# DJjjjhao/FIRA-ICSE

Measured on AMD Instinct MI355X. Metric: training commits/sec (FIRA default config), higher is better.
Workload: dtype f32; 1 GPU; BASELINE configs[1]: FIRA training step (fwd+bwd+Adam, dropout 0.1/0.2), batch 32 commits/GPU, fp32, 650-node graphs (mean nnz 1066/graph), vocab 24650; global_batch=32, parallelism=dp1

## Files before the change

fira_icse_amd/build.py:

```python
from __future__ import annotations

import os
import subprocess
import sys
from concurrent.futures import ThreadPoolExecutor

HERE = os.path.dirname(os.path.abspath(__file__))
CSRC = os.path.join(HERE, "csrc")
LIB = os.path.join(HERE, "libfira_hip.so")
SOURCES = ["gemm_f32.hip", "gemm_bf16.hip", "gemm_wgrad_panel.hip", "gemm_bf16_panel.hip", "gemm_small.hip", "spmm.hip", "spmm_dense.hip", "gcn_fused.hip", "comb_fused.hip", "head_x3.hip", "rowops.hip", "attention.hip", "copyhead.hip", "beam.hip", "engine.hip", "layout.cpp", "hostlists.cpp"]
HEADERS = ["common.h", "engine.h", "epilogue.h", "mfma_frag.h", "x3.h", os.path.join("..", "..", "include", "fira_hip.h")]
FLAGS = ["--offload-arch=gfx950", "-O3", "-std=c++17", "-fPIC", "-munsafe-fp-atomics", "-Wno-unused-result"]


def _hipcc() -> str:
    for cand in (os.environ.get("HIPCC"), "/opt/rocm/bin/hipcc", "hipcc"):
        if cand and (os.path.isabs(cand) and os.path.exists(cand) or not os.path.isabs(cand)):
            return cand
    raise RuntimeError("hipcc not found")


def build(force: bool = False, verbose: bool = False) -> str:
    objdir = os.path.join(HERE, "build")
    os.makedirs(objdir, exist_ok=True)
    hdr_time = max(os.path.getmtime(os.path.join(CSRC, h)) for h in HEADERS)
    hipcc = _hipcc()
    jobs = []
    for src in SOURCES:
        sp = os.path.join(CSRC, src)
        op = os.path.join(objdir, src + ".o")
        if force or not os.path.exists(op) or os.path.getmtime(op) < max(os.path.getmtime(sp), hdr_time):
            cmd = [hipcc] + FLAGS + (["-x", "hip"] if src.endswith(".cpp") else []) + ["-c", sp, "-o", op]
            jobs.append((src, cmd))

    def run(job):
        src, cmd = job
        if verbose:
            print(" ".join(cmd), flush=True)
        r = subprocess.run(cmd, capture_output=True, text=True)
        if r.returncode != 0:
            raise RuntimeError("hipcc failed on %s:\n%s" % (src, r.stderr[-4000:]))
        return src

    if jobs:
        with ThreadPoolExecutor(max_workers=min(8, len(jobs))) as ex:
            list(ex.map(run, jobs))
    objs = [os.path.join(objdir, s + ".o") for s in SOURCES]
    if jobs or not os.path.exists(LIB):
        cmd = [hipcc, "--offload-arch=gfx950", "-shared", "-fPIC", "-o", LIB] + objs
        r = subprocess.run(cmd, capture_output=True, text=True)
        if r.returncode != 0:
            raise RuntimeError("link failed:\n%s" % r.stderr[-4000:])
    return LIB


if __name__ == "__main__":
    print(build(force="--force" in sys.argv, verbose=True))
```

fira_icse_amd/csrc/comb_fused.hip:

```cpp
#include "engine.h"
#include "mfma_frag.h"
#include "epilogue.h"
#include "x3.h"

namespace fira {

constexpr int CF_TILE = 16;
constexpr int CF_TMAX = 2;
constexpr int CF_ROWS = CF_TILE * CF_TMAX;
constexpr int CF_WAVES = 16;
constexpr int CF_RPW = CF_ROWS / CF_WAVES;
constexpr int CF_GRID = 256;
constexpr size_t CF_LDS = 84 * 1024;

typedef float cf_acc __attribute__((ext_vector_type(4)));

struct CombFusedArgs {
    int n_rows;
    const float* Xc;
    const float *WqT, *WkT, *WoT;
    const float *bqk, *bo;
    const float* vtab;
    int ldv;
    const int32_t* mark;
    float *qk, *c;
    const float *gamma, *beta;
    float *sum, *y, *stats;
    const int32_t* y_rows;
    float p, inv_keep;
    uint64_t seed;
    uint32_t site_gate, site_out;
};

__device__ __forceinline__ int cf_off(int row, int quad) { return row * FIRA_D + ((quad ^ (row & 11)) << 2); }

__device__ __forceinline__ void cf_first_chunk(const float* __restrict__ W, unsigned wlane, float (&b0)[16]) {
    const rsrc_t rW = buf_rsrc(W, FIRA_D * FIRA_D * 4u);
#pragma unroll
    for (int s2 = 0; s2 < 16; ++s2)
        b0[s2] = __builtin_bit_cast(float, __builtin_amdgcn_raw_buffer_load_b32(rW, wlane, s2 * FIRA_D * 4, 0));
}

template <bool BF, int TM>
__device__ __forceinline__ void cf_product(const float* __restrict__ sm_u, const int (&a_off)[4], const float* __restrict__ W,
                                           unsigned wlane, int nt, float (&bx)[16], cf_acc (&acc)[TM],
                                           const float* __restrict__ Wnext = nullptr) {
    constexpr int NC = FIRA_D / 64;
    static_assert(NC % 2 == 0, "the buffer the last chunk leaves free is b[0]");
    const rsrc_t rW = buf_rsrc(W, FIRA_D * FIRA_D * 4u);
    const rsrc_t rN = buf_rsrc(Wnext ? Wnext : W, FIRA_D * FIRA_D * 4u);
    float b[2][16];
#pragma unroll
    for (int s2 = 0; s2 < 16; ++s2) b[0][s2] = bx[s2];
#pragma unroll
    for (int c = 0; c < NC; ++c) {
        if (c + 1 < NC) {
#pragma unroll
            for (int s2 = 0; s2 < 16; ++s2)
                b[(c + 1) & 1][s2] = __builtin_bit_cast(float, __builtin_amdgcn_raw_buffer_load_b32(
                                                                   rW, wlane, ((c + 1) * 64 + s2) * FIRA_D * 4, 0));
        } else if (Wnext) {
#pragma unroll
            for (int s2 = 0; s2 < 16; ++s2)
                b[0][s2] = __builtin_bit_cast(float, __builtin_amdgcn_raw_buffer_load_b32(rN, wlane, s2 * FIRA_D * 4, 0));
        }
        asm volatile("" ::: "memory");
#pragma unroll
        for (int tt = 0; tt < TM; ++tt) {
            if (tt < nt) {
                float af[16];
#pragma unroll
                for (int ii = 0; ii < 4; ++ii) {
                    const f32x4v q = *reinterpret_cast<const f32x4v*>(&sm_u[a_off[ii] + tt * (CF_TILE * FIRA_D) + c * 64]);
                    af[4 * ii] = q.x; af[4 * ii + 1] = q.y; af[4 * ii + 2] = q.z; af[4 * ii + 3] = q.w;
                }
                if constexpr (BF) {
#pragma unroll
                    for (int j = 0; j < 2; ++j) {
                        uint4 ua, ub;
                        ua.x = apk2(af[8 * j], af[8 * j + 1]); ua.y = apk2(af[8 * j + 2], af[8 * j + 3]);
                        ua.z = apk2(af[8 * j + 4], af[8 * j + 5]); ua.w = apk2(af[8 * j + 6], af[8 * j + 7]);
                        ub.x = apk2(b[c & 1][8 * j], b[c & 1][8 * j + 1]); ub.y = apk2(b[c & 1][8 * j + 2], b[c & 1][8 * j + 3]);
                        ub.z = apk2(b[c & 1][8 * j + 4], b[c & 1][8 * j + 5]); ub.w = apk2(b[c & 1][8 * j + 6], b[c & 1][8 * j + 7]);
                        acc[tt] = __builtin_amdgcn_mfma_f32_16x16x32_bf16(__builtin_bit_cast(abf16x8, ua),
                                                                          __builtin_bit_cast(abf16x8, ub), acc[tt], 0, 0, 0);
                    }
                } else {
#pragma unroll
                    for (int s2 = 0; s2 < 16; ++s2)
                        acc[tt] = __builtin_amdgcn_mfma_f32_16x16x4f32(af[s2], b[c & 1][s2], acc[tt], 0, 0, 0);
                }
            }
        }
        asm volatile("" ::: "memory");
    }
#pragma unroll
    for (int s2 = 0; s2 < 16; ++s2) bx[s2] = b[0][s2];
}

template <int NP>
__device__ __forceinline__ void cx_first(const uint16_t* __restrict__ Wx, unsigned xlane, uint4 (&b0)[3]) {
    const rsrc_t rW = buf_rsrc(Wx, 3u * (unsigned)GX_WPLANE);
#pragma unroll
    for (int pl = 0; pl < NP; ++pl)
        b0[pl] = __builtin_bit_cast(uint4, __builtin_amdgcn_raw_buffer_load_b128(rW, xlane, pl * (int)GX_WPLANE, 0));
}
template <int TM, int NP>
__device__ __forceinline__ void cx_product(const char* __restrict__ sm_p, size_t plane_bytes, int a_q, const uint16_t* __restrict__ Wx,
                                           unsigned xlane, int nt, uint4 (&bx)[3], cf_acc (&acc)[TM],
                                           const uint16_t* __restrict__ Wnext = nullptr) {
    const rsrc_t rW = buf_rsrc(Wx, 3u * (unsigned)GX_WPLANE);
    const rsrc_t rN = buf_rsrc(Wnext ? Wnext : Wx, 3u * (unsigned)GX_WPLANE);
    uint4 b[2][3];
#pragma unroll
    for (int pl = 0; pl < NP; ++pl) b[0][pl] = bx[pl];
#pragma unroll
    for (int ks = 0; ks < 8; ++ks) {
        if (ks + 1 < 8) {
#pragma unroll
            for (int pl = 0; pl < NP; ++pl)
                b[(ks + 1) & 1][pl] = __builtin_bit_cast(uint4, __builtin_amdgcn_raw_buffer_load_b128(
                                                                    rW, xlane, pl * (int)GX_WPLANE + (ks + 1) * 1024, 0));
        } else if (Wnext) {
#pragma unroll
            for (int pl = 0; pl < NP; ++pl)
                b[0][pl] = __builtin_bit_cast(uint4, __builtin_amdgcn_raw_buffer_load_b128(rN, xlane, pl * (int)GX_WPLANE, 0));
        }
        asm volatile("" ::: "memory");
#pragma unroll
        for (int tt = 0; tt < TM; ++tt) {
            if (tt < nt)
                gx_terms<NP>(acc[tt], sm_p + ((a_q ^ (ks << 6)) + tt * (CF_TILE * 512)), plane_bytes, b[ks & 1]);
        }
        asm volatile("" ::: "memory");
    }
#pragma unroll
    for (int pl = 0; pl < NP; ++pl) bx[pl] = b[0][pl];
}
constexpr size_t CX_PLANE = (size_t)CF_ROWS * 512;

template <bool BF, int NP = 0>
__global__ __launch_bounds__(CF_WAVES * 64) void comb_fused_fwd_kernel(const CombFusedArgs a) {
    constexpr bool X3 = NP > 0;
    constexpr int NPX = X3 ? NP : 3;
    extern __shared__ __attribute__((aligned(16))) float cf_lds[];
    float* const sm_u = cf_lds;
    char* const sm_p = reinterpret_cast<char*>(cf_lds);
    int* const sm_mark = reinterpret_cast<int*>(cf_lds + (X3 ? 3 * CX_PLANE / 4 : (size_t)CF_ROWS * FIRA_D));
    const int t = threadIdx.x, lane = t & 63, wave = t >> 6;
    const int l15 = lane & 15, kq = lane >> 4;
    const int wg = (blockIdx.x & 7) * (CF_GRID / 8) + (blockIdx.x >> 3);
    const int n_tiles = (a.n_rows + CF_TILE - 1) / CF_TILE;
    const int tq = n_tiles / CF_GRID, tr = n_tiles % CF_GRID;
    const int t_beg = wg * tq + min(wg, tr), t_cnt = tq + (wg < tr ? 1 : 0);
    if (t_cnt == 0) return;
    int a_off[4], d_off[4], r_off[CF_RPW];
// ... 343 lines not shown
    int nkb, kb_chunk, n_pairs;
    float* out;
    int ldo;
};
template <int NP>
__global__ __launch_bounds__(CF_WAVES * 64) void dgrad_x3_splitk_kernel(const DgradSplitKArgs a) {
    extern __shared__ __attribute__((aligned(16))) float cf_lds[];
    char* const sm_p = reinterpret_cast<char*>(cf_lds);
    const int t = threadIdx.x, lane = t & 63, wave = t >> 6;
    const int l15 = lane & 15, kq = lane >> 4;
    const int pi = blockIdx.x % a.n_pairs, ci = blockIdx.x / a.n_pairs;
    const int row0 = pi * CF_ROWS;
    const int row_end = min(a.n_rows, row0 + CF_ROWS);
    const int nt = (row_end - row0 + CF_TILE - 1) / CF_TILE;
    const int kb0 = ci * a.kb_chunk, kb1 = min(a.nkb, kb0 + a.kb_chunk);
    if (kb0 >= kb1) return;
    const int col = wave * 16 + l15;
    const unsigned xlane = gx_wlane(wave, lane);
    const int a_q = gx_frag_base(l15, kq);
    constexpr size_t WX = 3 * (size_t)FIRA_D * FIRA_D;
    uint4 bx3[3];
    cx_first<NP>(a.Wx + kb0 * WX, xlane, bx3);
    asm volatile("" ::: "memory");
    const float* arow[CF_RPW];
    bool live[CF_RPW];
    f32x4v x[CF_RPW];
    auto fetch = [&](int kb) {
#pragma unroll
        for (int i = 0; i < CF_RPW; ++i) {
            const int k = kb * FIRA_D + lane * 4;
            if (k + 3 < a.K) x[i] = *reinterpret_cast<const f32x4v*>(arow[i] + k);
            else x[i] = f32x4v{k < a.K ? arow[i][k] : 0.f, k + 1 < a.K ? arow[i][k + 1] : 0.f, k + 2 < a.K ? arow[i][k + 2] : 0.f, 0.f};
            if (!live[i]) x[i] = f32x4v{0.f, 0.f, 0.f, 0.f};
        }
    };
#pragma unroll
    for (int i = 0; i < CF_RPW; ++i) {
        const int row = row0 + wave * CF_RPW + i;
        live[i] = row < row_end;
        arow[i] = a.A + (size_t)min(row, a.n_rows - 1) * a.lda;
    }
    fetch(kb0);
    cf_acc acc[CF_TMAX];
#pragma unroll
    for (int tt = 0; tt < CF_TMAX; ++tt) acc[tt] = cf_acc{0.f, 0.f, 0.f, 0.f};
    for (int kb = kb0; kb < kb1; ++kb) {
#pragma unroll
        for (int i = 0; i < CF_RPW; ++i) gx_store_row4<NP>(sm_p, CX_PLANE, wave * CF_RPW + i, lane, x[i]);
        lds_barrier();   
        if (kb + 1 < kb1) fetch(kb + 1);
        cx_product<CF_TMAX, NP>(sm_p, CX_PLANE, a_q, a.Wx + kb * WX, xlane, nt, bx3, acc, kb + 1 < kb1 ? a.Wx + (kb + 1) * WX : nullptr);
        lds_barrier();   
    }
#pragma unroll
    for (int tt = 0; tt < CF_TMAX; ++tt) {
        if (tt < nt) {
#pragma unroll
            for (int r = 0; r < 4; ++r) {
                const int row = row0 + tt * CF_TILE + 4 * kq + r;
                if (row < row_end) unsafeAtomicAdd(a.out + (size_t)row * a.ldo + col, acc[tt][r]);
            }
        }
    }
}
int dgrad_x3_splitk(hipStream_t s, int M, int K, const float* A, int lda, const uint16_t* Wx, float* out, int ldo, bool one_plane) {
    if (M <= 0 || K <= 0) return 0;
    FIRA_REQUIRE(A && Wx && out && lda % 4 == 0 && (uintptr_t)A % 16 == 0 && lda >= K && ldo >= FIRA_D, "dgrad_x3_splitk: bad argument");
    ProfScope prof(s, PROF_GEMM, 2.0 * M * (double)K * FIRA_D, 4.0 * ((double)M * K + 2.0 * M * FIRA_D) + 6.0 * (double)K * FIRA_D);
    DgradSplitKArgs a{};
    a.n_rows = M; a.A = A; a.lda = lda; a.K = K; a.Wx = Wx; a.nkb = cdiv(K, FIRA_D); a.out = out; a.ldo = ldo;
    a.n_pairs = cdiv(M, CF_ROWS);
    const int chunks = std::max(1, std::min(cdiv(a.nkb, 4), cdiv(CF_GRID, a.n_pairs)));
    a.kb_chunk = cdiv(a.nkb, chunks);
    const int grid = a.n_pairs * cdiv(a.nkb, a.kb_chunk);
    const size_t lds = 3 * CX_PLANE + 256;
    if (one_plane) hipLaunchKernelGGL(dgrad_x3_splitk_kernel<1>, dim3(grid), dim3(CF_WAVES * 64), lds, s, a);
    else hipLaunchKernelGGL(dgrad_x3_splitk_kernel<3>, dim3(grid), dim3(CF_WAVES * 64), lds, s, a);
    FIRA_CHECK_LAUNCH("dgrad_x3_splitk");
    return 0;
}

int linear_x3(hipStream_t s, int M, const float* X, int ldx, const uint16_t* Wx, int nb, const float* bias, float* out, int ldo,
              bool one_plane) {
    if (M <= 0 || nb <= 0) return 0;
    FIRA_REQUIRE(X && Wx && out && ldx % 4 == 0 && (uintptr_t)X % 16 == 0, "linear_x3: bad argument");
    FIRA_REQUIRE((size_t)M * ldo * 4 < (1ull << 31), "linear_x3: %d x %d floats exceed the 2 GiB the kernel addresses", M, ldo);
    ProfScope prof(s, PROF_GEMM, 2.0 * M * (double)nb * FIRA_D * FIRA_D, 4.0 * ((double)M * FIRA_D + (double)M * nb * FIRA_D) + 6.0 * nb * FIRA_D * FIRA_D);
    LinearX3Args a{M, X, ldx, Wx, nb, bias, out, ldo};
    const size_t lds = 3 * CX_PLANE + 256;
    const int grid = linear_x3_grid(M);
    if (one_plane) hipLaunchKernelGGL(linear_x3_kernel<1>, dim3(grid), dim3(CF_WAVES * 64), lds, s, a);
    else hipLaunchKernelGGL(linear_x3_kernel<3>, dim3(grid), dim3(CF_WAVES * 64), lds, s, a);
    FIRA_CHECK_LAUNCH("linear_x3");
    return 0;
}

int comb_fused_fwd(hipStream_t s, int n_rows, const float* Xc, const float* WqT, const float* WkT, const float* WoT,
                   const float* bqk, const float* bo, const float* vtab, int ldv, const int32_t* mark, float* qk, float* c,
                   const float* gamma, const float* beta, float* sum, float* y, const int32_t* y_rows, float* stats,
                   float dropout, uint64_t seed, uint32_t site_gate, uint32_t site_out, int bf16, const uint16_t* Wx) {
    if (n_rows <= 0) return 0;
    FIRA_REQUIRE(Xc && WqT && WkT && WoT && bqk && bo && vtab && mark && qk && c && gamma && beta && sum && y && stats,
                 "comb_fused_fwd: null pointer argument");
    FIRA_REQUIRE((uintptr_t)Xc % 16 == 0 && (uintptr_t)sum % 16 == 0 && (uintptr_t)y % 16 == 0 && (uintptr_t)WqT % 16 == 0,
                 "comb_fused_fwd: rows must be 16-byte aligned");
    FIRA_REQUIRE((size_t)n_rows * 2 * FIRA_D * 4 < (1ull << 31), "comb_fused_fwd: %d rows exceed the 2 GiB the kernel addresses", n_rows);
    ProfScope prof(s, PROF_COMB, 3.0 * 2.0 * n_rows * FIRA_D * FIRA_D, 4.0 * n_rows * FIRA_D * (1.0 + 2.0 + 1.0 + 1.0 + 1.0));
    CombFusedArgs a{};
    a.n_rows = n_rows; a.Xc = Xc; a.WqT = WqT; a.WkT = WkT; a.WoT = WoT; a.bqk = bqk; a.bo = bo; a.vtab = vtab; a.ldv = ldv;
    a.mark = mark; a.qk = qk; a.c = c; a.gamma = gamma; a.beta = beta; a.sum = sum; a.y = y; a.stats = stats; a.y_rows = y_rows;
    a.p = dropout; a.inv_keep = dropout > 0.f ? 1.0f / (1.0f - dropout) : 1.0f; a.seed = seed; a.site_gate = site_gate;
    a.site_out = site_out;
    static const int attr = [] {
        hipError_t e = hipFuncSetAttribute((const void*)comb_fused_fwd_kernel<false>, hipFuncAttributeMaxDynamicSharedMemorySize, (int)CF_LDS);
        if (e == hipSuccess)
            e = hipFuncSetAttribute((const void*)comb_fused_fwd_kernel<true>, hipFuncAttributeMaxDynamicSharedMemorySize, (int)CF_LDS);
        if (e == hipSuccess)
            e = hipFuncSetAttribute((const void*)comb_fused_fwd_kernel<false, 3>, hipFuncAttributeMaxDynamicSharedMemorySize, (int)CF_LDS);
        if (e == hipSuccess)
            e = hipFuncSetAttribute((const void*)comb_fused_fwd_kernel<false, 1>, hipFuncAttributeMaxDynamicSharedMemorySize, (int)CF_LDS);
        return e == hipSuccess ? 0 : set_err("comb_fused: cannot raise the dynamic LDS limit: %s", hipGetErrorString(e));
    }();
    if (attr) return attr;
    if (Wx) {
        a.WqT = reinterpret_cast<const float*>(Wx);
        if (bf16) hipLaunchKernelGGL((comb_fused_fwd_kernel<false, 1>), dim3(CF_GRID), dim3(CF_WAVES * 64), CF_LDS, s, a);
        else hipLaunchKernelGGL((comb_fused_fwd_kernel<false, 3>), dim3(CF_GRID), dim3(CF_WAVES * 64), CF_LDS, s, a);
    } else
    if (bf16) hipLaunchKernelGGL(comb_fused_fwd_kernel<true>, dim3(CF_GRID), dim3(CF_WAVES * 64), CF_LDS, s, a);
    else hipLaunchKernelGGL(comb_fused_fwd_kernel<false>, dim3(CF_GRID), dim3(CF_WAVES * 64), CF_LDS, s, a);
    FIRA_CHECK_LAUNCH("comb_fused_fwd");
    return 0;
}

constexpr int CB_TMAX = 1;
constexpr int CB_ROWS = CF_TILE * CB_TMAX;
constexpr int CB_RPW = CB_ROWS / CF_WAVES;

struct CombFusedBwdArgs {
    int n_rows;
    float* dG;
    const int32_t* rows;
    const float *sum, *stats, *gamma;
    const float *Wo, *Wqk;
    const float* qk;
    const float* vtab;
    int ldv;
    const int32_t* mark;
    float *dYc, *dqk;
    float *part_ln, *part_v;
    float p, inv_keep;
    uint64_t seed;
    uint32_t site_gate, site_out;
};

constexpr size_t CBX_PLANE = (size_t)CB_ROWS * 512;
constexpr size_t CB_LDS_X3 = 100 * 1024;
constexpr size_t CB_LDS_X3_2 = 2 * 3 * (size_t)2 * CF_TILE * 512 + 256 + 48 * 1024 + 1024;
template <bool BF, int NP = 0, int TM = 1>
__global__ __launch_bounds__(CF_WAVES * 64) void comb_fused_bwd_kernel(const CombFusedBwdArgs a) {
    constexpr int CB_TMAX = TM, CB_ROWS = CF_TILE * TM, CB_RPW = CB_ROWS / CF_WAVES;
    constexpr size_t CBX_PLANE = (size_t)CB_ROWS * 512;
    constexpr bool X3 = NP > 0;
    constexpr int NPX = X3 ? NP : 3;
    extern __shared__ __attribute__((aligned(16))) float cf_lds[];
    constexpr size_t PANEL = X3 ? 3 * CBX_PLANE / 4 : (size_t)CB_ROWS * FIRA_D;
    float* const sm_u = cf_lds;
    float* const sm_w = cf_lds + PANEL;
    char* const sm_p1 = reinterpret_cast<char*>(sm_u);
    char* const sm_p2 = reinterpret_cast<char*>(sm_w);
    int* const sm_mark = reinterpret_cast<int*>(cf_lds + 2 * PANEL);
    float* const red = cf_lds + 2 * PANEL + 64;
    float* const redv = red + CF_WAVES * 2 * FIRA_D;
    const int t = threadIdx.x, lane = t & 63, wave = t >> 6;
    const int l15 = lane & 15, kq = lane >> 4;
    const int wg = (blockIdx.x & 7) * (CF_GRID / 8) + (blockIdx.x >> 3);
    const int n_tiles = (a.n_rows + CF_TILE - 1) / CF_TILE;
    const int tq = n_tiles / CF_GRID, tr = n_tiles % CF_GRID;
    const int t_beg = wg * tq + min(wg, tr), t_cnt = tq + (wg < tr ? 1 : 0);
    int a_off[4], d_off[4], r_off[CB_RPW];
#pragma unroll
    for (int ii = 0; ii < 4; ++ii) a_off[ii] = cf_off(l15, kq * 4 + ii);
#pragma unroll
    for (int r = 0; r < 4; ++r) d_off[r] = cf_off(4 * kq + r, (wave * 16 + l15) >> 2) + (l15 & 3);
#pragma unroll
    for (int i = 0; i < CB_RPW; ++i) r_off[i] = cf_off(wave * CB_RPW + i, lane);
    const int col = wave * 16 + l15;
    const unsigned wlane = (unsigned)((kq * 16) * FIRA_D + col) * 4u;
    const rsrc_t rQK = buf_rsrc(a.qk, (unsigned)((size_t)a.n_rows * 2 * FIRA_D * 4));
    const rsrc_t rDQK = buf_rsrc(a.dqk, (unsigned)((size_t)a.n_rows * 2 * FIRA_D * 4));
    const float is = 1.0f / 5.656854249492381f;
    const unsigned xlane = gx_wlane(wave, lane);
    const int a_q = gx_frag_base(l15, kq);
    const uint16_t* const WTx = reinterpret_cast<const uint16_t*>(a.Wo);
    constexpr size_t WX = 3 * (size_t)FIRA_D * FIRA_D;
    *reinterpret_cast<f32x4v*>(&red[wave * 2 * FIRA_D + lane * 4]) = f32x4v{0.f, 0.f, 0.f, 0.f};
    *reinterpret_cast<f32x4v*>(&red[wave * 2 * FIRA_D + FIRA_D + lane * 4]) = f32x4v{0.f, 0.f, 0.f, 0.f};
#pragma unroll
    for (int m = 0; m < 4; ++m) redv[(kq * 4 + m) * FIRA_D + col] = 0.f;

    for (int pass = 0; pass < t_cnt; pass += CB_TMAX) {
        const int nt = min(CB_TMAX, t_cnt - pass);
        const int row0 = (t_beg + pass) * CF_TILE;
        const int row_end = min(a.n_rows, row0 + nt * CF_TILE);
        float bx[16];
        uint4 bx3[3];
        if constexpr (X3) cx_first<NPX>(WTx + 2 * WX, xlane, bx3);
        else cf_first_chunk(a.Wo, wlane, bx);
        asm volatile("" ::: "memory");
        const int rbase = row0 + wave * CB_RPW;
        int nr[CB_RPW];
        f32x4v ds[CB_RPW];
        {
            f32x4v d[CB_RPW], sv[CB_RPW];
            float mean[CB_RPW], rstd[CB_RPW];
            const f32x4v gam = *reinterpret_cast<const f32x4v*>(a.gamma + lane * 4);
#pragma unroll
            for (int i = 0; i < CB_RPW; ++i) nr[i] = a.rows[min(rbase + i, a.n_rows - 1)];
            if (t < CB_ROWS) sm_mark[t] = a.mark[min(row0 + t, a.n_rows - 1)];
#pragma unroll
            for (int i = 0; i < CB_RPW; ++i) {
                const int row = min(rbase + i, a.n_rows - 1);
                d[i] = *reinterpret_cast<const f32x4v*>(a.dG + (size_t)nr[i] * FIRA_D + lane * 4);
                sv[i] = *reinterpret_cast<const f32x4v*>(a.sum + (size_t)row * FIRA_D + lane * 4);
                mean[i] = a.stats[2 * row];
                rstd[i] = a.stats[2 * row + 1];
            }
#pragma unroll
            for (int i = 0; i < CB_RPW; ++i) {
                const bool live = rbase + i < row_end;
                if (!live) { d[i] = f32x4v{0.f, 0.f, 0.f, 0.f}; rstd[i] = 0.f; }
                const f32x4v xh = (sv[i] - mean[i]) * rstd[i];
                *reinterpret_cast<f32x4v*>(&red[wave * 2 * FIRA_D + lane * 4]) += d[i] * xh;
                *reinterpret_cast<f32x4v*>(&red[wave * 2 * FIRA_D + FIRA_D + lane * 4]) += d[i];
                const f32x4v h = d[i] * gam;
                const f32x4v hx = h * xh;
                const float m1 = wave_sum(h.x + h.y + h.z + h.w) * (1.0f / FIRA_D);
                const float m2 = wave_sum(hx.x + hx.y + hx.z + hx.w) * (1.0f / FIRA_D);
                ds[i] = (h - m1 - xh * m2) * rstd[i];
                f32x4v o4 = ds[i];
                if (a.p > 0.f) {
                    const uint32_t e0 = (uint32_t)(rbase + i) * FIRA_D + lane * 4;
                    o4.x *= dropout_scale(a.seed, a.site_out, e0 + 0, a.p, a.inv_keep);
                    o4.y *= dropout_scale(a.seed, a.site_out, e0 + 1, a.p, a.inv_keep);
                    o4.z *= dropout_scale(a.seed, a.site_out, e0 + 2, a.p, a.inv_keep);
                    o4.w *= dropout_scale(a.seed, a.site_out, e0 + 3, a.p, a.inv_keep);
                }
                if constexpr (X3) gx_store_row4<NPX>(sm_p1, CBX_PLANE, wave * CB_RPW + i, lane, o4);
                else *reinterpret_cast<f32x4v*>(&sm_u[r_off[i]]) = o4;
                if (live) *reinterpret_cast<f32x4v*>(a.dYc + (size_t)(rbase + i) * FIRA_D + lane * 4) = o4;
            }
        }
        lds_barrier();   
        float qs[CB_TMAX][4], ks[CB_TMAX][4];
        auto load_qk = [&]() {
#pragma unroll
            for (int tt = 0; tt < CB_TMAX; ++tt)
#pragma unroll
                for (int r = 0; r < 4; ++r) {
                    const int row = row0 + tt * CF_TILE + 4 * kq + r;
                    const unsigned o2 = row < row_end ? ((unsigned)row * 2 * FIRA_D + col) * 4u : FIRA_OOB;
                    qs[tt][r] = __builtin_bit_cast(float, __builtin_amdgcn_raw_buffer_load_b32(rQK, o2, 0, 0));
                    ks[tt][r] = __builtin_bit_cast(float, __builtin_amdgcn_raw_buffer_load_b32(rQK, o2, FIRA_D * 4, 0));
                }
            asm volatile("" ::: "memory");
        };
        if constexpr (!BF) load_qk();
        cf_acc ac[CB_TMAX];
#pragma unroll
        for (int tt = 0; tt < CB_TMAX; ++tt) ac[tt] = cf_acc{0.f, 0.f, 0.f, 0.f};
        if constexpr (X3) cx_product<CB_TMAX, NPX>(sm_p1, CBX_PLANE, a_q, WTx + 2 * WX, xlane, nt, bx3, ac, WTx);
        else
        cf_product<BF, CB_TMAX>(sm_u, a_off, a.Wo, wlane, nt, bx, ac, a.Wqk);
        if constexpr (BF) load_qk();
        lds_barrier();
#pragma unroll
        for (int tt = 0; tt < CB_TMAX; ++tt) {
            if (tt < nt) {
#pragma unroll
                for (int r = 0; r < 4; ++r) {
                    const int rl = tt * CF_TILE + 4 * kq + r, row = row0 + rl;
                    const bool live = row < row_end;
                    float dc = ac[tt][r];
                    if (a.p > 0.f) dc *= dropout_scale(a.seed, a.site_gate, (uint32_t)row * FIRA_D + col, a.p, a.inv_keep);
                    const int m = sm_mark[rl];
                    const float v = a.vtab[(size_t)m * a.ldv + col];
                    const float q = qs[tt][r], k = ks[tt][r];
                    float g0, g1;
                    gate_elem(q, k, v, g0, g1);
                    const float dg0 = dc * k, dg1 = dc * v;
                    const float dot = g0 * dg0 + g1 * dg1;
                    const float da = g0 * (dg0 - dot), db = g1 * (dg1 - dot);
                    const float dq = live ? (da * k + db * v) * is : 0.f;
                    const float dk = live ? dc * g0 + da * q * is : 0.f;
                    const float dv = live ? dc * g1 + db * q * is : 0.f;
                    const unsigned o2 = live ? ((unsigned)row * 2 * FIRA_D + col) * 4u : FIRA_OOB;
                    __builtin_amdgcn_raw_buffer_store_b32(__builtin_bit_cast(unsigned, dq), rDQK, o2, 0, 0);
                    __builtin_amdgcn_raw_buffer_store_b32(__builtin_bit_cast(unsigned, dk), rDQK, o2, FIRA_D * 4, 0);
                    redv[(kq * 4 + m) * FIRA_D + col] += dv;
                    if constexpr (X3) {
                        gx_store_elem<NPX>(sm_p1, CBX_PLANE, rl, col, dq);
                        gx_store_elem<NPX>(sm_p2, CBX_PLANE, rl, col, dk);
                    } else {
                    sm_u[d_off[r] + tt * (CF_TILE * FIRA_D)] = dq;
                    sm_w[d_off[r] + tt * (CF_TILE * FIRA_D)] = dk;
                    }
                }
            }
        }
        lds_barrier();   
        cf_acc ax[CB_TMAX];
#pragma unroll
        for (int tt = 0; tt < CB_TMAX; ++tt) ax[tt] = cf_acc{0.f, 0.f, 0.f, 0.f};
        if constexpr (X3) {
            cx_product<CB_TMAX, NPX>(sm_p1, CBX_PLANE, a_q, WTx, xlane, nt, bx3, ax, WTx + WX);
            cx_product<CB_TMAX, NPX>(sm_p2, CBX_PLANE, a_q, WTx + WX, xlane, nt, bx3, ax);
        } else {
        cf_product<BF, CB_TMAX>(sm_u, a_off, a.Wqk, wlane, nt, bx, ax, a.Wqk + (size_t)FIRA_D * FIRA_D);
        cf_product<BF, CB_TMAX>(sm_w, a_off, a.Wqk + (size_t)FIRA_D * FIRA_D, wlane, nt, bx, ax);
        }
        lds_barrier();   
#pragma unroll
        for (int tt = 0; tt < CB_TMAX; ++tt) {
            if (tt < nt) {
#pragma unroll
                for (int r = 0; r < 4; ++r) sm_u[d_off[r] + tt * (CF_TILE * FIRA_D)] = ax[tt][r];
            }
        }
        lds_barrier();   
#pragma unroll
        for (int i = 0; i < CB_RPW; ++i) {
            if (rbase + i >= row_end) continue;
            const f32x4v x = *reinterpret_cast<const f32x4v*>(&sm_u[r_off[i]]);
            *reinterpret_cast<f32x4v*>(a.dG + (size_t)nr[i] * FIRA_D + lane * 4) = ds[i] + x;
        }
        lds_barrier();
    }
    lds_barrier();   
    if (t < 2 * FIRA_D) {
        float acc = 0.f;
#pragma unroll
        for (int w = 0; w < CF_WAVES; ++w) acc += red[w * 2 * FIRA_D + t];
        a.part_ln[(size_t)blockIdx.x * 2 * FIRA_D + t] = acc;
    }
    {
        const int m = t >> 8, cc = t & 255;
        a.part_v[(size_t)blockIdx.x * 4 * FIRA_D + t] = (redv[(0 * 4 + m) * FIRA_D + cc] + redv[(1 * 4 + m) * FIRA_D + cc]) +
                                                        (redv[(2 * 4 + m) * FIRA_D + cc] + redv[(3 * 4 + m) * FIRA_D + cc]);
    }
}

int comb_fused_bwd_parts() { return CF_GRID; }
int comb_fused_bwd(hipStream_t s, int n_rows, float* dG, const int32_t* rows, const float* sum, const float* stats,
                   const float* gamma, const float* Wo, const float* Wqk, const float* qk, const float* vtab, int ldv,
                   const int32_t* mark, float* dYc, float* dqk, float* part_ln, float* part_v, float dropout, uint64_t seed,
                   uint32_t site_gate, uint32_t site_out, int bf16, const uint16_t* WTx) {
    if (n_rows <= 0) return 0;
    FIRA_REQUIRE(dG && rows && sum && stats && gamma && Wo && Wqk && qk && vtab && mark && dYc && dqk && part_ln && part_v,
                 "comb_fused_bwd: null pointer argument");
    FIRA_REQUIRE((uintptr_t)dG % 16 == 0 && (uintptr_t)sum % 16 == 0 && (uintptr_t)dYc % 16 == 0 && (uintptr_t)Wo % 16 == 0,
                 "comb_fused_bwd: rows must be 16-byte aligned");
    FIRA_REQUIRE((size_t)n_rows * 2 * FIRA_D * 4 < (1ull << 31), "comb_fused_bwd: %d rows exceed the 2 GiB the kernel addresses", n_rows);
    ProfScope prof(s, PROF_COMB, 3.0 * 2.0 * n_rows * FIRA_D * FIRA_D, 4.0 * n_rows * FIRA_D * (2.0 + 2.0 + 1.0 + 2.0 + 1.0));
    CombFusedBwdArgs a{};
    a.n_rows = n_rows; a.dG = dG; a.rows = rows; a.sum = sum; a.stats = stats; a.gamma = gamma; a.Wo = Wo; a.Wqk = Wqk; a.qk = qk;
    a.vtab = vtab; a.ldv = ldv; a.mark = mark; a.dYc = dYc; a.dqk = dqk; a.part_ln = part_ln; a.part_v = part_v;
    a.p = dropout; a.inv_keep = dropout > 0.f ? 1.0f / (1.0f - dropout) : 1.0f; a.seed = seed; a.site_gate = site_gate;
    a.site_out = site_out;
    static const int attr = [] {
        hipError_t e = hipFuncSetAttribute((const void*)comb_fused_bwd_kernel<false>, hipFuncAttributeMaxDynamicSharedMemorySize, (int)CF_LDS);
        if (e == hipSuccess)
            e = hipFuncSetAttribute((const void*)comb_fused_bwd_kernel<true>, hipFuncAttributeMaxDynamicSharedMemorySize, (int)CF_LDS);
        if (e == hipSuccess)
            e = hipFuncSetAttribute((const void*)comb_fused_bwd_kernel<false, 3>, hipFuncAttributeMaxDynamicSharedMemorySize, (int)CB_LDS_X3);
        if (e == hipSuccess)
            e = hipFuncSetAttribute((const void*)comb_fused_bwd_kernel<false, 1>, hipFuncAttributeMaxDynamicSharedMemorySize, (int)CB_LDS_X3);
        if (e == hipSuccess)
            e = hipFuncSetAttribute((const void*)comb_fused_bwd_kernel<false, 3, 2>, hipFuncAttributeMaxDynamicSharedMemorySize, (int)CB_LDS_X3_2);
        if (e == hipSuccess)
            e = hipFuncSetAttribute((const void*)comb_fused_bwd_kernel<false, 1, 2>, hipFuncAttributeMaxDynamicSharedMemorySize, (int)CB_LDS_X3_2);
        return e == hipSuccess ? 0 : set_err("comb_fused: cannot raise the dynamic LDS limit: %s", hipGetErrorString(e));
    }();
    if (attr) return attr;
    if (WTx) {
        a.Wo = reinterpret_cast<const float*>(WTx);
        const int n_tiles = (n_rows + CF_TILE - 1) / CF_TILE;
        if (n_tiles > CF_GRID) {
            if (bf16) hipLaunchKernelGGL((comb_fused_bwd_kernel<false, 1, 2>), dim3(CF_GRID), dim3(CF_WAVES * 64), CB_LDS_X3_2, s, a);
            else hipLaunchKernelGGL((comb_fused_bwd_kernel<false, 3, 2>), dim3(CF_GRID), dim3(CF_WAVES * 64), CB_LDS_X3_2, s, a);
        } else
        if (bf16) hipLaunchKernelGGL((comb_fused_bwd_kernel<false, 1>), dim3(CF_GRID), dim3(CF_WAVES * 64), CB_LDS_X3, s, a);
        else hipLaunchKernelGGL((comb_fused_bwd_kernel<false, 3>), dim3(CF_GRID), dim3(CF_WAVES * 64), CB_LDS_X3, s, a);
    } else
    if (bf16) hipLaunchKernelGGL(comb_fused_bwd_kernel<true>, dim3(CF_GRID), dim3(CF_WAVES * 64), CF_LDS, s, a);
    else hipLaunchKernelGGL(comb_fused_bwd_kernel<false>, dim3(CF_GRID), dim3(CF_WAVES * 64), CF_LDS, s, a);
    FIRA_CHECK_LAUNCH("comb_fused_bwd");
    return 0;
}

__global__ __launch_bounds__(256) void transpose256_table_kernel(const TransposeTable tab) {
    __shared__ float tile[64][65];
    const float* src = tab.src[blockIdx.z];
    float* dst = tab.dst[blockIdx.z];
    const int r0 = blockIdx.y * 64, c0 = blockIdx.x * 64;
    const int tx = threadIdx.x & 63, ty = threadIdx.x >> 6;
    for (int r = ty; r < 64; r += 4) tile[r][tx] = src[(size_t)(r0 + r) * FIRA_D + c0 + tx];
    __syncthreads();
    for (int r = ty; r < 64; r += 4) dst[(size_t)(c0 + r) * FIRA_D + r0 + tx] = tile[tx][r];
}
int transpose256_table(hipStream_t s, const TransposeTable& tab) {
    if (tab.n <= 0) return 0;
    hipLaunchKernelGGL(transpose256_table_kernel, dim3(FIRA_D / 64, FIRA_D / 64, tab.n), dim3(256), 0, s, tab);
    FIRA_CHECK_LAUNCH("transpose256_table");
    return 0;
}

}

extern "C" {
int fira_linear_dgrad_x3(void* stream, int M, int K, const float* dy, int lddy, const uint16_t* wt_planes, float* dx, int lddx,
                         int accumulate, int dtype) {
    FIRA_REQUIRE(dy && wt_planes && dx && M > 0 && K > 0 && K % FIRA_D == 0 && lddx >= FIRA_D, "fira_linear_dgrad_x3: bad argument");
    FIRA_REQUIRE(dtype == FIRA_F32X3 || dtype == FIRA_BF16X1, "fira_linear_dgrad_x3: dtype must be FIRA_F32X3 or FIRA_BF16X1");
    return fira::linear_x3_kacc((hipStream_t)stream, M, dy, lddy, wt_planes, K / FIRA_D, dx, lddx, accumulate != 0,
                                dtype == FIRA_BF16X1);
}
size_t fira_dgrad_x3_splitk_planes_bytes(int K) { return (size_t)((K + FIRA_D - 1) / FIRA_D) * 3 * FIRA_D * FIRA_D * sizeof(uint16_t); }
int fira_dgrad_x3_splitk(void* stream, int M, int K, const float* dy, int lddy, const float* W, uint16_t* planes_ws, float* dx,
                         int lddx, int dtype) {
    FIRA_REQUIRE(dy && W && planes_ws && dx && M > 0 && K > 0, "fira_dgrad_x3_splitk: bad argument");
    FIRA_REQUIRE(dtype == FIRA_F32X3 || dtype == FIRA_BF16X1, "fira_dgrad_x3_splitk: dtype must be FIRA_F32X3 or FIRA_BF16X1");
    const bool one = dtype == FIRA_BF16X1;
    const int rc = fira::split_planes_t((hipStream_t)stream, W, K, planes_ws, one);
    return rc ? rc : fira::dgrad_x3_splitk((hipStream_t)stream, M, K, dy, lddy, planes_ws, dx, lddx, one);
}
int fira_linear_x3(void* stream, int M, int N, const float* x, int ldx, const uint16_t* w_planes, const float* bias, float* out,
                   int ldo, int dtype) {
    FIRA_REQUIRE(x && w_planes && out && M > 0 && N > 0 && N % FIRA_D == 0 && ldo >= N, "fira_linear_x3: bad argument");
    FIRA_REQUIRE(dtype == FIRA_F32X3 || dtype == FIRA_BF16X1, "fira_linear_x3: dtype must be FIRA_F32X3 or FIRA_BF16X1");
    return fira::linear_x3((hipStream_t)stream, M, x, ldx, w_planes, N / FIRA_D, bias, out, ldo, dtype == FIRA_BF16X1);
}
int fira_combination_block_bwd(void* stream, int n_rows, float* dG, const int32_t* rows, const float* sum, const float* stats,
                               const float* gamma, const float* Wo, const float* Wqk, const float* qk, const float* vtab, int ldv,
                               const int32_t* mark, float* dYc, float* dqk, float* dgamma, float* dbeta, float* dvtab, int lddv,
                               float* part, float dropout, uint64_t seed, uint32_t site_gate, uint32_t site_out, int dtype) {
    FIRA_REQUIRE(dropout >= 0.f && dropout < 1.f, "fira_combination_block_bwd: dropout must be in [0,1)");
    FIRA_REQUIRE(dtype >= FIRA_F32 && dtype <= FIRA_BF16X1, "fira_combination_block_bwd: dtype must be FIRA_F32, FIRA_BF16, FIRA_F32X3 or FIRA_BF16X1");
    FIRA_REQUIRE(dgamma && dbeta && dvtab && part, "fira_combination_block_bwd: null pointer argument");
    const int nb = fira::comb_fused_bwd_parts();
    float* part_ln = part;
    float* part_v = part + (size_t)nb * 2 * FIRA_D;
    if (int rc = fira::comb_fused_bwd((hipStream_t)stream, n_rows, dG, rows, sum, stats, gamma, Wo, Wqk, qk, vtab, ldv, mark, dYc, dqk,
                                      part_ln, part_v, dropout, seed, site_gate, site_out, dtype == FIRA_BF16 || dtype == FIRA_BF16X1,
                                      dtype >= FIRA_F32X3 ? reinterpret_cast<const uint16_t*>(Wo) : nullptr))
        return rc;
    if (n_rows <= 0) return 0;
    fira::RedTable tab;
    tab.e[0] = fira::RedEntry{dgamma, part_ln, FIRA_D, nb, 2 * FIRA_D};
    tab.e[1] = fira::RedEntry{dbeta, part_ln + FIRA_D, FIRA_D, nb, 2 * FIRA_D};
    for (int k = 0; k < 4; ++k) tab.e[2 + k] = fira::RedEntry{dvtab + (size_t)k * lddv, part_v + k * FIRA_D, FIRA_D, nb, 4 * FIRA_D};
    tab.n = 6;
    return fira::deferred_reduce((hipStream_t)stream, tab);
}
int fira_combination_block_bwd_part_floats(void) { return fira::comb_fused_bwd_parts() * 6 * FIRA_D; }
int fira_combination_block_fwd(void* stream, int n_rows, const float* Xc, const float* WqT, const float* WkT, const float* WoT,
                               const float* bqk, const float* bo, const float* vtab, int ldv, const int32_t* mark, float* qk,
                               float* c, const float* gamma, const float* beta, float* sum, float* y, const int32_t* y_rows,
                               float* stats, float dropout, uint64_t seed, uint32_t site_gate, uint32_t site_out, int dtype) {
    FIRA_REQUIRE(dropout >= 0.f && dropout < 1.f, "fira_combination_block_fwd: dropout must be in [0,1)");
    FIRA_REQUIRE(dtype >= FIRA_F32 && dtype <= FIRA_BF16X1, "fira_combination_block_fwd: dtype must be FIRA_F32, FIRA_BF16, FIRA_F32X3 or FIRA_BF16X1");
    return fira::comb_fused_fwd((hipStream_t)stream, n_rows, Xc, WqT, WkT, WoT, bqk, bo, vtab, ldv, mark, qk, c, gamma, beta, sum,
                                y, y_rows, stats, dropout, seed, site_gate, site_out, dtype == FIRA_BF16 || dtype == FIRA_BF16X1,
                                dtype >= FIRA_F32X3 ? reinterpret_cast<const uint16_t*>(WqT) : nullptr);
}
}
```

fira_icse_amd/csrc/engine.h:

```cpp
#pragma once
#include "common.h"
#include <string>
#include <vector>

namespace fira {

int gemm_f32(hipStream_t s, int tA, int tB, int M, int N, int K, const float* A, int lda, const float* B, int ldb,
             float* C, int ldc, const float* bias, int flags, int splitk);
int gemm_f32_ex(hipStream_t s, int tA, int tB, int M, int N, int K, const float* A, int lda, const float* B, int ldb,
                float* C, int ldc, const float* bias, int flags, int splitk, float* colsum,
                const int32_t* c_rows = nullptr, const float* relu_mask = nullptr);
int gemm_bf16_ex(hipStream_t s, int tA, int tB, int M, int N, int K, const float* A, int lda, const float* B, int ldb,
                 float* C, int ldc, const float* bias, int flags, int splitk, float* colsum,
                 const int32_t* c_rows = nullptr, const float* relu_mask = nullptr);
struct ShadowEntry { int64_t offset; int rows, cols, pitch_t; int64_t offset_t; };
constexpr int SHADOW_MAX = 64;
struct ShadowTable {
    int n = 0;
    int64_t wbt_elems = 0;
    int tile_start[SHADOW_MAX + 1] = {0};
    ShadowEntry e[SHADOW_MAX];
};
int weight_shadows(hipStream_t s, const ShadowTable& tab, const float* P, uint16_t* Wb, uint16_t* WbT);
int gemm_bf16_wb_ex(hipStream_t s, int M, int N, int K, const float* A, int lda, const uint16_t* Bb, int ldb, float* C,
                    int ldc, const float* bias, int flags, int splitk, const int32_t* c_rows = nullptr,
                    const float* relu_mask = nullptr);
int gemm_bf16_group_add_wgrad(hipStream_t s, int M, int N, int K, const float* A, int lda, const float* B, int ldb,
                              float* C, int ldc, float* colsum, int max_split = 0);
int gemm_bf16_group_flush(hipStream_t s);
bool gemm_bf16_takes(int M, int N, int K);
void gemm_bf16_group_reset();
bool gemm_bf16_group_full();
bool gemm_wgrad_panel_takes(int M, int N, int K, const float* A, int lda, const float* B, int ldb, int ldc);
void gemm_wgrad_panel_reset();
bool gemm_wgrad_panel_full();
int gemm_wgrad_panel_pending();
int gemm_wgrad_panel_add(int M, int N, int K, const float* A, int lda, const float* B, int ldb, float* C, int ldc, float* colsum);
int gemm_wgrad_panel_flush(hipStream_t s, int np);
void gemm_wgrad_panel_scratch(float* buf, size_t n_floats);
int gemm_wgrad_panel(hipStream_t s, int np, int M, int N, int K, const float* A, int lda, const float* B, int ldb, float* C,
                     int ldc, float* colsum);
int gemm_group_add_wgrad(hipStream_t s, int M, int N, int K, const float* A, int lda, const float* B, int ldb, float* C,
                         int ldc, float* colsum, int max_split = 0);
int gemm_group_flush(hipStream_t s);
void gemm_group_reset();
bool gemm_group_full();
void gemm_set_pad_stream(hipStream_t s);
struct EpiRes;
bool gemm_tile32_takes(int tB, int M, int N, int K, const float* A, int lda, const float* B, int ldb);
bool gemm_tile32_try(hipStream_t s, int tB, int M, int N, int K, const float* A, int lda, const float* B, int ldb,
                     float* C, int ldc, const float* bias, int flags, int* rc, const int32_t* c_rows,
                     const float* relu_mask, const int32_t* a_rows, const EpiRes* er);
bool gemm_tile32_ln_try(hipStream_t s, int M, int N, const float* S, int lds, const float* W, const float* bias, float* Y,
                        int ldy, int flags, const float* gamma, const float* beta, float* x_out, float* stats_out, int* rc);
int gemm_tile32_lnb_blocks(int M);
bool gemm_tile32_lnb_try(hipStream_t s, int M, int N, const float* dy, const float* W, int ldw, float* dX, int lddx,
                         const float* relu_mask, const float* sum, const float* stats, const float* gamma, float* ds,
                         float* dx_drop, float* part, float dropout, uint64_t seed, uint32_t site, int* rc,
                         uint32_t idx0 = 0);
bool gemm_small_try(hipStream_t s, int tA, int tB, int M, int N, int K, const float* A, int lda, const float* B, int ldb,
                    float* C, int ldc, const float* bias, int flags, int* rc, const int32_t* c_rows = nullptr,
                    const float* relu_mask = nullptr);
int csr_spmm(hipStream_t s, int n_rows, const int32_t* rowptr, const int32_t* col, const float* val, const float* X,
             int ldx, float* Y, int ldy, int graph_rows, int variant);
int csr_spmm_ex(hipStream_t s, int n_rows, const int32_t* rowptr, const int32_t* col, const float* val, const float* X,
                int ldx, float* Y, int ldy, int graph_rows, int variant, int accum, float* rowsum);
int gcn_fused_fwd(hipStream_t s, int n_rows, const int32_t* rowptr, const int32_t* col, const float* val, const float* X,
                  const float* Wk, const float* bias, const float* r1_col, const float* gamma, const float* beta, float* sum,
                  float* y, float* stats, float* rowsum_out, const int32_t* slot2, float* y2, float dropout, uint64_t seed,
                  uint32_t site, int bf16, const uint16_t* Wx = nullptr);
int gcn_fused_bwd(hipStream_t s, int n_rows, const int32_t* rowptr, const int32_t* col, const float* val, const float* dY,
                  const float* Wk, float* u_out, float* acc_out, int bf16, const uint16_t* Wx = nullptr);
int gcn_split_planes(hipStream_t s, int n, const float* const* src, uint16_t* const* dst);
size_t head_logits_x3_scratch_elems(int R);
int head_logits_x3(hipStream_t s, int R, int V, const float* x, int ldx, const float* W, const float* bias, float* out, int ldo,
                   uint16_t* xplanes);
int transpose256(hipStream_t s, int nl, const float* W, float* Wt);
int linear_x3(hipStream_t s, int M, const float* X, int ldx, const uint16_t* Wx, int nb, const float* bias, float* out, int ldo,
              bool one_plane);
int split_planes_t(hipStream_t s, const float* W, int V, uint16_t* planes, bool one_plane);
int dgrad_x3_splitk(hipStream_t s, int M, int K, const float* A, int lda, const uint16_t* Wx, float* out, int ldo, bool one_plane);
int linear_x3_kacc(hipStream_t s, int M, const float* A, int lda, const uint16_t* Wx, int nkb, float* out, int ldo, bool accum,
                   bool one_plane);
int comb_fused_fwd(hipStream_t s, int n_rows, const float* Xc, const float* WqT, const float* WkT, const float* WoT,
                   const float* bqk, const float* bo, const float* vtab, int ldv, const int32_t* mark, float* qk, float* c,
                   const float* gamma, const float* beta, float* sum, float* y, const int32_t* y_rows, float* stats,
                   float dropout, uint64_t seed, uint32_t site_gate, uint32_t site_out, int bf16, const uint16_t* Wx = nullptr);
int comb_fused_bwd_parts();
int comb_fused_bwd(hipStream_t s, int n_rows, float* dG, const int32_t* rows, const float* sum, const float* stats,
                   const float* gamma, const float* Wo, const float* Wqk, const float* qk, const float* vtab, int ldv,
                   const int32_t* mark, float* dYc, float* dqk, float* part_ln, float* part_v, float dropout, uint64_t seed,
                   uint32_t site_gate, uint32_t site_out, int bf16, const uint16_t* WTx = nullptr);
struct TransposeTable { int n = 0; const float* src[24]; float* dst[24]; };
int transpose256_table(hipStream_t s, const TransposeTable& tab);
int embed_gather_fwd(hipStream_t s, int B, int L, const int32_t* idx, const float* table, const float* pos, float* out,
                     int out_bstride, int out_off);
int embed_grouped_bwd(hipStream_t s, int n_items, const int32_t* item_tok, const int32_t* item_ptr, const int32_t* rows,
                      float* dtable, const float* dnode);
int embed_list_bwd_small(hipStream_t s, int n, const int32_t* rows, const int32_t* ids, float* dtable, const float* dnode,
                         int table_rows);
int embed_gather_bwd(hipStream_t s, int B, int L, const int32_t* idx, float* dtable, const float* dout,
                     int out_bstride, int out_off, int padding_idx);
int embed_gather_bwd_small(hipStream_t s, int B, int L, const int32_t* idx, float* dtable, const float* dout,
                           int out_bstride, int out_off, int padding_idx, int table_rows);
int combination_fwd(hipStream_t s, int M, const float* qk, const float* vtab, int ldv, const int32_t* mark, float* out,
                    float dropout, uint64_t seed, uint32_t site);
int combination_bwd(hipStream_t s, int M, const float* qk, const float* vtab, int ldv, const int32_t* mark,
                    const float* dout, float* dqk, float* dvtab, int lddv, float dropout, uint64_t seed, uint32_t site,
                    float* part = nullptr);
int combination_bwd_blocks(int M);
struct RedEntry { float* dst; const float* src; int width, n_part, stride; };
constexpr int RED_MAX = 96;
struct RedTable {
    int n = 0;
    int wg_start[RED_MAX + 1] = {0};
    RedEntry e[RED_MAX];
};
int deferred_reduce(hipStream_t s, RedTable& tab);
int add_layernorm_fwd(hipStream_t s, int M, float* x, const float* res, const float* gamma, const float* beta,
                      float* y, float* stats, float dropout, uint64_t seed, uint32_t site, const int32_t* y_rows, const float* r1_row = nullptr,
                      const float* r1_col = nullptr,
                      const int32_t* slot2 = nullptr, float* y2 = nullptr,
                      uint32_t idx0 = 0);
bool gemm_bf16_k256_try(hipStream_t s, int M, int N, int K, const float* A, int lda, const uint16_t* Bb, int ldb, float* C,
                        int ldc, const float* bias, int flags, const int32_t* c_rows, const float* relu_mask, int* rc);
bool linear_ln_bf16_try(hipStream_t s, int M, int K, const float* X, int ldx, const uint16_t* Wb, int ldb, const float* bias,
                        const float* res, const float* gamma, const float* beta, float* sum, float* y, float* stats,
                        float dropout, uint64_t seed, uint32_t site, const int32_t* y_rows, const float* r1_row,
                        const float* r1_col, int* rc, bool force = false);
int add_layernorm_bwd(hipStream_t s, int M, const float* dy, const float* sum, const float* stats, const float* gamma,
                      float* ds, float* dx_drop, float* dgamma, float* dbeta, float dropout, uint64_t seed,
                      uint32_t site, const int32_t* rows = nullptr,
                      float* part = nullptr,
                      const float* row_w = nullptr, uint32_t idx0 = 0);
int add_layernorm_bwd_blocks(int M);
int gcn_bias_unfold(hipStream_t s, const float* W2, const float* b1, const float* dc, float* dW2, float* db1);
struct UnfoldEntry { const float *W2, *b1, *dc; float *dW2, *db1; };
struct UnfoldTable { int n = 0; UnfoldEntry e[16]; };
int gcn_bias_unfold_all(hipStream_t s, const UnfoldTable& tab);
int gcn_fold_weights(hipStream_t s, int n_layers, const float* const* W2, const float* const* W1, const float* const* b1,
                     float* W21, float* W21t, float* c21);
int gcn_unfold_products(hipStream_t s, int n_layers, const float* const* dW21, const float* const* W1, const float* const* W2,
                        float* const* dW1, float* const* dW2);
int colsum(hipStream_t s, int M, int N, const float* X, int ldx, float* out, const float* row_weight = nullptr);
int rank2_rows(hipStream_t s, int M, const float* g, const float* w, float* out);
int prep(hipStream_t s, int B, int L, int S, int T, const int32_t* sou, const int32_t* sub, const int32_t* tar,
         int32_t* mem_valid, int32_t* tar_valid, float* pos_code, float* pos_tar, int R, const int32_t* rows,
         int32_t* compact_row, int32_t* iota, float* loss_sum = nullptr, int32_t* n_tok = nullptr,
         int Nc = 0, const int32_t* code_rows = nullptr, int Cc = 0, int32_t* code_slot = nullptr,
         const int32_t* mem_rows = nullptr, int Mc = 0, int32_t* mem_slot = nullptr,
         const int32_t* dec_off = nullptr, int32_t* row_bt = nullptr, int32_t* rows_c = nullptr,
         const int32_t* mem_dst = nullptr, int32_t* mem_off = nullptr, int32_t* mem_valid_c = nullptr);
struct AdamRowsView;
int embed_rows_fwd(hipStream_t s, int R, int T, const int32_t* row_bt, const int32_t* idx, const float* table,
                   const float* pos, float* out, const AdamRowsView* vw = nullptr);
int embed_rows_bwd(hipStream_t s, int R, const int32_t* row_bt, const int32_t* idx, float* dtable, const float* dout,
                   int padding_idx);
int node_features(hipStream_t s, int Nc, const int32_t* node_rows, int N, int L, int S, const int32_t* sou,
                  const int32_t* sub, const int32_t* ast, const float* emb, const float* ast_emb, const float* pos_code,
                  float* X, const int32_t* slot2 = nullptr, float* X2 = nullptr,
                  const AdamRowsView* vw = nullptr);
int rows_move(hipStream_t s, int mode, int R, int W, float* out, const float* in, const int32_t* src, const int32_t* dst);
int rows_move_ld(hipStream_t s, int mode, int R, int W, float* out, int ld_out, const float* in, int ld_in,
                 const int32_t* src, const int32_t* dst);
int rows_gather_idx(hipStream_t s, int R, float* compact, const float* src, const int32_t* rows);
int rows_scatter_add_idx(hipStream_t s, int R, const float* compact, float* dst, const int32_t* rows);
int fill_pos_tables(hipStream_t s, int L, float* pos_code, int T, float* pos_tar);
int tar_mask(hipStream_t s, int n, const int32_t* tar, int32_t* valid);
int permute_cache(hipStream_t s, int nl, int BR, int T, int len, const int32_t* parent, const float* ksrc,
                  const float* vsrc, float* kdst, float* vdst, const int32_t* hist_src, int32_t* hist_dst);
int mark_history(hipStream_t s, int BR, int T, int step, const int32_t* tokens, int32_t* hist);
int decode_embed(hipStream_t s, int BR, int T, int step, const int32_t* tokens, const float* table, const float* pos_row,
                 float* x, int32_t* hist);

int attention_fwd(hipStream_t s, int B, int H, int Tq, int Tk, const float* Q, int ldq, const float* K, int ldk,
                  const float* V, int ldv, const int32_t* key_valid, int causal, int q_pos0, float* O, int ldo,
                  const int32_t* q_off = nullptr, int self_kv = 0,
                  int bf16 = 0,
                  const int32_t* k_off = nullptr);
int attention_fwd_ex(hipStream_t s, int B, int H, int Tq, int Tk, const float* Q, int ldq, const float* K, int ldk,
                     const float* V, int ldv, const int32_t* key_valid, int causal, int q_pos0, float* O, int ldo,
                     int kb, int kvb, int qpk, const int32_t* q_off = nullptr, int self_kv = 0, int bf16 = 0,
                     const int32_t* k_off = nullptr);
int decode_attention(hipStream_t s, int BR, int H, int Tk, const float* Q, int ldq, const float* K, int ldk,
                     const float* V, int ldv, const int32_t* key_valid, float* O, int ldo, int kb, int kvb, int qpk,
                     const float* Knew = nullptr, const float* Vnew = nullptr, int ldn = 0, float* Kc_out = nullptr,
                     float* Vc_out = nullptr, const int32_t* k_off = nullptr);
int decode_self_block(hipStream_t s, int BR, int Tk, int T, const float* qkv, float* Kc, float* Vc, const int32_t* hist,
                      const float* WoT, const float* bo, const float* xres, const float* gamma, const float* beta,
                      const float* WqT, const float* bq, float* xa, float* qc);
int decode_attention_kv16(hipStream_t s, int BR, int H, int Tk, const float* Q, int ldq, const uint16_t* K, int ldk,
                          const uint16_t* V, int ldv, const int32_t* key_valid, float* O, int ldo, int kb, int kvb, int qpk,
                          const int32_t* k_off = nullptr);
int rows_to_bf16(hipStream_t s, int64_t n, const float* in, uint16_t* out);
int rows_from_bf16(hipStream_t s, int64_t n, const uint16_t* in, float* out);
int attention_bwd(hipStream_t s, int B, int H, int Tq, int Tk, const float* Q, int ldq, const float* K, int ldk,
                  const float* V, int ldv, const int32_t* key_valid, int causal, int q_pos0, const float* O, int ldo,
                  const float* dO, int lddo, float* dQ, int lddq, float* dK, int lddk, float* dV, int lddv,
                  const int32_t* q_off = nullptr, int self_kv = 0, int bf16 = 0, const int32_t* k_off = nullptr);
int copy_score_fwd(hipStream_t s, int B, int T, int S, const float* src, const float* tgt, const float* w,
                   const float* bias, float* score);
int copy_score_fwd_ex(hipStream_t s, int B, int T, int S, const float* src, const float* tgt, const float* w,
                      const float* bias, float* score, int qpk, const int32_t* mem_valid,
                      const int32_t* tar_label = nullptr, int V = 0,
                      const int32_t* t_off = nullptr);
int copy_score_bwd_ex(hipStream_t s, int B, int T, int S, const float* src, const float* tgt, const float* w,
                      const float* dscore, float* dsrc, float* dtgt, float* dw, float* dbias, const int32_t* mem_valid,
                      float* part = nullptr, const int32_t* t_off = nullptr);
int copy_score_bwd_blocks(int B, int S);
constexpr int COPY_PART_STRIDE = 264;
int decode_dist(hipStream_t s, int R, int V, int S, const float* logits, int ldl, const float* score,
                const int32_t* mem_valid, int qpk, const float* gate_logits, float* dist, int32_t* best_id,
                float* best_p, const float* x = nullptr, const float* wp = nullptr, const float* bp = nullptr);
int inv_count(hipStream_t s, const int32_t* n_tok, float* out);
int row_topk(hipStream_t s, int R, int V, int k, const float* logits, int ldl, int32_t* ids, float* vals);
int copy_score_bwd(hipStream_t s, int B, int T, int S, const float* src, const float* tgt, const float* w,
                   const float* dscore, float* dsrc, float* dtgt, float* dw, float* dbias);
int head_loss(hipStream_t s, int BT, int T, int V, int S, const int32_t* compact_row, float* logits, int ldl,
              float* score, const int32_t* mem_valid, float* gate_logits, const int32_t* tar_label, float* loss_sum,
              int32_t* n_tok, int32_t* argmax_out, int want_grad,
              const int32_t* row_bt = nullptr);
int adam_step(hipStream_t s, int64_t n, float* p, const float* g, float* m, float* v, float lr, float beta1,
              float beta2, float eps, int step, const float* scale_ptr, int scale_is_count = 0);
int adam_step_mb(hipStream_t s, int64_t n, float* p, const float* g0, const float* g1, float* m, float* v, float lr,
                 float beta1, float beta2, float eps, int step, const int32_t* n0, const int32_t* n1);
constexpr int ADAM_ROWS_K = 32;
struct AdamRowsHist { float bc1[ADAM_ROWS_K], bc2s[ADAM_ROWS_K]; };
struct AdamRowsTables { float *p, *m, *v; int64_t off[2]; int rows[2]; int32_t* last; };
struct AdamRowsView {
    const float *m = nullptr, *v = nullptr;
    const int32_t* last = nullptr;
    int to = 0;
    float lr = 0.f, beta1 = 0.f, beta2 = 0.f, eps = 0.f, gz = 0.f;
    AdamRowsHist h;
};
AdamRowsView adam_rows_view(const AdamRowsTables& tb, int table, float lr, float beta1, float beta2, float eps, int to);
struct AdamRowsLists { int n_lists; int end[4]; int table[4]; const int32_t* ids[4]; };
int adam_rows_step(hipStream_t s, const AdamRowsTables& tb, const float* g, float lr, float beta1, float beta2, float eps,
                   int step, const int32_t* n0, const float* count, int tables = 3);
int adam_rows_catchup(hipStream_t s, const AdamRowsTables& tb, const AdamRowsLists* ls, float lr, float beta1, float beta2,
                      float eps, int to);

struct ParamInfo {
    std::string name;
    int64_t offset = -1, numel = 0;
// ... 24 lines not shown
```

fira_icse_amd/csrc/engine.hip:

```cpp
#include "engine.h"
#include <hip/hip_ext.h>
#include "epilogue.h"
#include <stdlib.h>
#include <map>
#include <mutex>

namespace fira {

static int64_t shadow_wbt_elems(const Layout& L);

struct Arena {
    char* base;
    size_t used = 0;
    explicit Arena(void* b) : base((char*)b) {}
    template <typename T>
    T* get(size_t n) {
        size_t bytes = (n * sizeof(T) + 255) / 256 * 256;
        T* p = base ? (T*)(base + used) : nullptr;
        used += bytes;
        return p;
    }
    float* f(size_t n) { return get<float>(n); }
};

struct EncSave {
    float *Xc, *qk, *c, *s1, *st1, *Z, *s2, *st2;
};
struct DecSave {
    float *qkv, *ao, *s_a, *st_a, *x_a, *qc, *ao2, *s_c, *st_c, *x_c, *h, *s_f, *st_f, *x_f;
};

struct EncGrad {
    float *dY2, *dYc, *dqk;
};
struct DecGrad {
    float *dYf, *dh, *dYc, *dq, *dYs, *dqkv;
};


static constexpr int KV_ROW_PAD = 64;

struct Plan {
    int B, NB, CB, MB, TB, N, L, S, A, T, V, ldl, nl, F;
    int kvp;
    float *pos_code, *pos_tar;
    int32_t *mem_valid, *tar_valid, *compact_row, *iota, *code_slot, *mem_slot, *row_bt, *rows_c;
    int32_t *mem_off, *mem_valid_c;
    std::vector<float*> X;
    std::vector<EncSave> enc;
    std::vector<DecSave> dec;
    std::vector<EncGrad> encg;
    std::vector<DecGrad> decg;
    float *vtab_all, *H, *mem, *mem_c, *src_c, *x0, *kv_all, *src, *tgt, *score, *gate, *dec_c, *logits;
    float *W21, *c21, *rsum;
    float *W21t;
    uint16_t *W21x = nullptr, *W21tx = nullptr;
    uint16_t *WcX = nullptr, *WcTX = nullptr;
    uint16_t* WkvX = nullptr;
    float* WkvT = nullptr;
    uint16_t* WkvTX = nullptr;
    uint16_t* WoutTX = nullptr;
    uint16_t *xh_planes = nullptr;
    float *WcT;
    float *dW21, *dc21;
    float *inv_ntok;
    float *dXa, *dXb, *dNB2, *dCB_a, *dvtab_all;
    float *zero_beg = nullptr, *zero_end = nullptr;
    uint16_t *wb = nullptr, *wbt = nullptr;
    uint16_t *w21b = nullptr, *w21bt = nullptr;
    float* red_buf = nullptr;
    size_t red_cap = 0;
    float* panel_scratch = nullptr;
    size_t panel_floats = 0;
    float *dmem_c, *dsrc, *dsrc_c, *dtgt, *dkv_all, *ddec, *ddec_c, *dT_a, *dT_c;

    size_t build(void* ws, const fira_dims& d, int B_, bool training) {
        Arena a(ws);
        B = B_; L = d.sou_len; S = d.sub_len; A = d.ast_len; T = d.tar_len; V = d.vocab; nl = d.n_layer; F = d.d_ff;
        N = L + S + A;
        NB = B * N; CB = B * L; MB = B * (L + S); TB = B * T;
        ldl = (V + 63) / 64 * 64;
        const size_t D = FIRA_D;
        pos_code = a.f((size_t)L * D);
        pos_tar = a.f((size_t)T * D);
        mem_valid = a.get<int32_t>((size_t)MB);
        tar_valid = a.get<int32_t>((size_t)TB);
        compact_row = a.get<int32_t>((size_t)TB);
        iota = a.get<int32_t>((size_t)TB);
        row_bt = a.get<int32_t>((size_t)TB);
        rows_c = a.get<int32_t>((size_t)TB);
        code_slot = a.get<int32_t>((size_t)NB);
        mem_slot = a.get<int32_t>((size_t)NB);
        mem_off = a.get<int32_t>((size_t)B + 1);
        mem_valid_c = a.get<int32_t>((size_t)MB);
        inv_ntok = a.f(64);
        {
            const Layout* lay = get_layout(&d);
            const size_t tot = lay ? (size_t)lay->total : 0;
            wb = a.get<uint16_t>(tot);
            wbt = a.get<uint16_t>((lay ? (size_t)shadow_wbt_elems(*lay) : 0) + 64);
            w21b = a.get<uint16_t>((size_t)nl * D * D);
            w21bt = a.get<uint16_t>((size_t)nl * D * D + 64);
        }
        X.resize(nl + 1);
        for (int l = 0; l <= nl; ++l) X[l] = a.f((size_t)NB * D);
        enc.resize(nl);
        for (int l = 0; l < nl; ++l) {
            EncSave& e = enc[l];
            e.Xc = a.f((size_t)CB * D); e.qk = a.f((size_t)CB * 2 * D); e.c = a.f((size_t)CB * D);
            e.s1 = a.f((size_t)CB * D); e.st1 = a.f((size_t)CB * 2);
            e.Z = a.f((size_t)NB * D); e.s2 = a.f((size_t)NB * D); e.st2 = a.f((size_t)NB * 2);
        }
        vtab_all = a.f((size_t)4 * nl * D);
        W21 = a.f((size_t)nl * D * D); c21 = a.f((size_t)nl * D); rsum = a.f((size_t)NB);
        W21t = a.f((size_t)nl * D * D);
        W21x = a.get<uint16_t>((size_t)nl * 3 * D * D);
        W21tx = a.get<uint16_t>((size_t)nl * 3 * D * D);
        WcX = a.get<uint16_t>((size_t)nl * 9 * D * D);
        WcTX = a.get<uint16_t>((size_t)nl * 9 * D * D);
        WkvX = a.get<uint16_t>((size_t)nl * 6 * D * D);
        WkvT = a.f((size_t)nl * 2 * D * D);
        WkvTX = a.get<uint16_t>((size_t)nl * 6 * D * D);
        WoutTX = a.get<uint16_t>((size_t)cdiv(V, D) * 3 * D * D);
        xh_planes = a.get<uint16_t>(head_logits_x3_scratch_elems(TB));
        WcT = a.f((size_t)nl * 3 * D * D);
        H = a.f((size_t)NB * D);
        mem = a.f((size_t)MB * D);
        mem_c = a.f((size_t)MB * D);
        src_c = a.f((size_t)MB * D);
        x0 = a.f((size_t)TB * D);
        kvp = nl * 2 * D + KV_ROW_PAD;
        kv_all = a.f((size_t)MB * kvp);
        dec.resize(nl);
        for (int l = 0; l < nl; ++l) {
            DecSave& e = dec[l];
            e.qkv = a.f((size_t)TB * 3 * D); e.ao = a.f((size_t)TB * D); e.s_a = a.f((size_t)TB * D);
            e.st_a = a.f((size_t)TB * 2); e.x_a = a.f((size_t)TB * D); e.qc = a.f((size_t)TB * D);
            e.ao2 = a.f((size_t)TB * D); e.s_c = a.f((size_t)TB * D); e.st_c = a.f((size_t)TB * 2);
            e.x_c = a.f((size_t)TB * D); e.h = a.f((size_t)TB * F); e.s_f = a.f((size_t)TB * D);
            e.st_f = a.f((size_t)TB * 2); e.x_f = a.f((size_t)TB * D);
        }
        src = a.f((size_t)MB * D); tgt = a.f((size_t)TB * D);
        score = a.f((size_t)TB * (L + S)); gate = a.f((size_t)TB * 2);
        dec_c = a.f((size_t)TB * D); logits = a.f((size_t)TB * ldl);
        if (training) {
            dXa = a.f((size_t)NB * D); dXb = a.f((size_t)NB * D); dNB2 = a.f((size_t)NB * D);
            dCB_a = a.f((size_t)CB * D);
            red_cap = (size_t)nl * ((size_t)cdiv(NB, 16) * 4 * D + (size_t)cdiv(CB, 16) * 2 * D)
                    + (size_t)3 * nl * cdiv(TB, 16) * 2 * D
                    + (size_t)nl * std::max((size_t)cdiv(CB, 16) * 4 * D, (size_t)comb_fused_bwd_parts() * 6 * D + 64)
                    + (size_t)cdiv(L + S, 16) * B * COPY_PART_STRIDE + 4096;
            red_buf = a.f(red_cap);
            panel_floats = (size_t)320 * 256 * 256;
            panel_scratch = a.f(panel_floats);
            zero_beg = (float*)a.get<char>(0);
            dvtab_all = a.f((size_t)4 * nl * D);
            dW21 = a.f((size_t)nl * D * D + (size_t)nl * D); dc21 = dW21 + (size_t)nl * D * D;
            dtgt = a.f((size_t)TB * D);
            ddec_c = a.f((size_t)TB * D);
            zero_end = (float*)a.get<char>(0);
            dmem_c = a.f((size_t)MB * D); dsrc = a.f((size_t)MB * D); dsrc_c = a.f((size_t)MB * D);
            dkv_all = a.f((size_t)MB * kvp);
            ddec = a.f((size_t)TB * D);
            dT_a = a.f((size_t)TB * D); dT_c = a.f((size_t)TB * D);
            encg.resize(nl);
            decg.resize(nl);
            for (int l = 0; l < nl; ++l) {
                EncGrad& g = encg[l];
                g.dY2 = a.f((size_t)NB * D); g.dYc = a.f((size_t)CB * D);
                g.dqk = a.f((size_t)CB * 2 * D);
                DecGrad& h = decg[l];
                h.dYf = a.f((size_t)TB * D); h.dh = a.f((size_t)TB * F); h.dYc = a.f((size_t)TB * D);
                h.dq = a.f((size_t)TB * D); h.dYs = a.f((size_t)TB * D); h.dqkv = a.f((size_t)TB * 3 * D);
            }
        }
        return a.used;
    }
};

#define TRY(x)                 \
    do {                       \
        if (int e__ = (x)) return e__; \
    } while (0)

static int zero(hipStream_t s, void* p, size_t bytes) {
    hipError_t e = hipMemsetAsync(p, 0, bytes, s);
    if (e != hipSuccess) return set_err("hipMemsetAsync: %s", hipGetErrorString(e));
    return 0;
}

static thread_local int g_dtype = 0;
static thread_local int g_lanes = 1;
struct DtypeScope {
    int prev;
    explicit DtypeScope(int d) : prev(g_dtype) { g_dtype = d; }
    ~DtypeScope() { g_dtype = prev; }
};
static thread_local const float* g_P = nullptr;
static thread_local int64_t g_total = 0;
static thread_local const uint16_t* g_Wb = nullptr;
static thread_local const uint16_t* g_WbT = nullptr;
static thread_local const ShadowTable* g_tab = nullptr;
static thread_local const float* g_W21 = nullptr;
static thread_local int64_t g_W21n = 0;
static thread_local const uint16_t* g_W21b = nullptr;
static thread_local const uint16_t* g_W21bT = nullptr;

static const ShadowTable* shadow_table(const Layout& L) {
    static std::mutex mu;
    static std::map<const Layout*, ShadowTable*> cache;
    std::lock_guard<std::mutex> g(mu);
    auto it = cache.find(&L);
    if (it != cache.end()) return it->second;
    ShadowTable* t = new ShadowTable();
    const int D = FIRA_D;
    auto add = [&](int64_t off, int rows, int cols) {
        if (t->n == SHADOW_MAX) return;
        const int pitch = (rows + 7) / 8 * 8;
        t->e[t->n] = ShadowEntry{off, rows, cols, pitch, t->wbt_elems};
        t->wbt_elems += ((int64_t)cols * pitch + 63) / 64 * 64;
        t->tile_start[t->n + 1] = t->tile_start[t->n] + cdiv(rows, 64) * cdiv(cols, 64);
        ++t->n;
    };
    for (int l = 0; l < L.d.n_layer; ++l) {
        add(L.enc[l].wqk, 2 * D, D);
        add(L.enc[l].wo, D, D);
        add(L.dec[l].wqkv, 3 * D, D);
        add(L.dec[l].wo_s, D, D);
        add(L.dec[l].wq_c, D, D);
        add(L.dec[l].wo_c, D, D);
        add(L.dec[l].w1, L.d.d_ff, D);
        add(L.dec[l].w2, D, L.d.d_ff);
    }
    add(L.wkv_all, L.d.n_layer * 2 * D, D);
    add(L.wout, L.d.vocab, D);
    add(L.ws, D, D);
    add(L.wt, D, D);
    cache[&L] = t;
    return t;
}
static int64_t shadow_wbt_elems(const Layout& L) { return shadow_table(L)->wbt_elems; }
struct ShadowScope {
    ShadowScope(const float* P, int64_t total, const uint16_t* wb, const uint16_t* wbt, const ShadowTable* tab) {
        g_P = P; g_total = total; g_Wb = wb; g_WbT = wbt; g_tab = tab;
    }
    ~ShadowScope() {
        g_P = nullptr; g_total = 0; g_Wb = nullptr; g_WbT = nullptr; g_tab = nullptr;
        g_W21 = nullptr; g_W21n = 0; g_W21b = nullptr; g_W21bT = nullptr;
    }
};
static bool shadow_of(const float* W, bool transposed, const uint16_t** out, int* ld) {
    if (!g_Wb || !g_tab) return false;
    if (g_W21b && W >= g_W21 && W < g_W21 + g_W21n) {
        const int64_t off = W - g_W21;
        if (off % (FIRA_D * FIRA_D)) return false;
        *out = (transposed ? g_W21bT : g_W21b) + off;
        *ld = FIRA_D;
        return true;
    }
    if (W < g_P || W >= g_P + g_total) return false;
    const int64_t off = W - g_P;
    for (int i = 0; i < g_tab->n; ++i) {
        const ShadowEntry& e = g_tab->e[i];
        if (off < e.offset || off >= e.offset + (int64_t)e.rows * e.cols) continue;
        const int64_t rel = off - e.offset;
        if (rel % e.cols) return false;
        if (!transposed) { *out = g_Wb + off; *ld = e.cols; }
        else { *out = g_WbT + e.offset_t + rel / e.cols; *ld = e.pitch_t; }
        return true;
    }
    return false;
}
static inline int gemm_any(hipStream_t s, int tA, int tB, int M, int N, int K, const float* A, int lda, const float* B,
                           int ldb, float* C, int ldc, const float* bias, int flags, int splitk, float* colsum,
                           const int32_t* c_rows = nullptr, const float* relu_mask = nullptr) {
    if (g_dtype == 1) {
        const uint16_t* wb;
        int ldw;
        if (!tA && !colsum && gemm_bf16_takes(M, N, K) && lda % 4 == 0 && shadow_of(B, !tB, &wb, &ldw) &&
            (tB ? ldb == K : ldb == N) && ldw % 8 == 0 && ((uintptr_t)wb % 16) == 0)
            return gemm_bf16_wb_ex(s, M, N, K, A, lda, wb, ldw, C, ldc, bias, flags, splitk, c_rows, relu_mask);
        return gemm_bf16_ex(s, tA, tB, M, N, K, A, lda, B, ldb, C, ldc, bias, flags, splitk, colsum, c_rows, relu_mask);
    }
    return gemm_f32_ex(s, tA, tB, M, N, K, A, lda, B, ldb, C, ldc, bias, flags, splitk, colsum, c_rows, relu_mask);
}

static inline int linear(hipStream_t s, int M, int N, int K, const float* X, int ldx, const float* W, const float* b,
                         float* Y, int ldy, int flags = 0) {
    return gemm_any(s, 0, 1, M, N, K, X, ldx, W, K, Y, ldy, b, flags, 0, nullptr);
}
static inline int linear_ln(hipStream_t s, int M, int K, const float* X, int ldx, const float* W, const float* b,
                            const float* res, const float* gamma, const float* beta, float* sum, float* y, float* stats,
                            float p_drop, uint64_t seed, uint32_t st, const int32_t* y_rows = nullptr,
                            const float* r1_row = nullptr, const float* r1_col = nullptr,
                            const int32_t* slot2 = nullptr, float* y2 = nullptr, int n2 = 0, const int32_t* rows2 = nullptr,
                            uint32_t idx0 = 0) {
    bool fused = false;
    int rc = 0;
    if (g_dtype != 0 && idx0 == 0 && g_lanes == 1) {
        const uint16_t* wb;
        int ldw;
// ... 72 lines not shown
    hipEvent_t ev() {
        if (!pool.empty()) { hipEvent_t e = pool.back(); pool.pop_back(); return e; }
        hipEvent_t e = nullptr;
        (void)hipEventCreate(&e);
        return e;
    }
    void report() {
        (void)hipDeviceSynchronize();
        std::vector<std::pair<int, std::pair<double, int>>> acc;
        for (auto& r : recs) {
            float ms = 0.f;
            if (hipEventElapsedTime(&ms, r.a, r.b) != hipSuccess) ms = 0.f;
            bool found = false;
            for (auto& q : acc) if (q.first == r.line) { q.second.first += ms; q.second.second++; found = true; }
            if (!found) acc.push_back({r.line, {ms, 1}});
            pool.push_back(r.a); pool.push_back(r.b);
        }
        recs.clear();
        fprintf(stderr, "[fira wait probe] over %d calls, us per call the caller's stream spent at each wait (engine.hip line: us):", calls);
        double tot = 0;
        for (auto& q : acc) { fprintf(stderr, "  %d: %.1f", q.first, 1e3 * q.second.first / calls); tot += 1e3 * q.second.first / calls; }
        fprintf(stderr, "  | total %.1f\n", tot);
        calls = 0;
    }
};
static WaitProbe& wait_probe() { static thread_local WaitProbe w; return w; }
static int stream_wait_probed(hipStream_t main_s, hipEvent_t e, int line) {
    WaitProbe& w = wait_probe();
    if (!w.enabled()) return hipStreamWaitEvent(main_s, e, 0) == hipSuccess ? 0 : 1;
    WaitProbe::Rec r{line, w.ev(), w.ev()};
    (void)hipEventRecord(r.a, main_s);
    const bool ok = hipStreamWaitEvent(main_s, e, 0) == hipSuccess;
    (void)hipEventRecord(r.b, main_s);
    w.recs.push_back(r);
    return ok ? 0 : 1;
}

static int side_join(hipStream_t main_s, int line = 0) {
    SideStream& sd = side();
    hipEvent_t e = sd.ev();
    if (hipEventRecord(e, sd.stream) != hipSuccess || stream_wait_probed(main_s, e, line))
        return set_err("side stream join failed");
    return 0;
}

static inline bool side_on() { SideStream& sd = side(); return sd.stream && sd.enabled; }
static int aux_fork(hipStream_t main_s) {
    SideStream& sd = side();
    hipEvent_t e = sd.ev();
    if (hipEventRecord(e, main_s) != hipSuccess || hipStreamWaitEvent(sd.aux, e, 0) != hipSuccess)
        return set_err("aux stream fork failed");
    return 0;
}
static int side_mark(hipEvent_t* out) {
    SideStream& sd = side();
    hipEvent_t e = sd.ev();
    if (hipEventRecord(e, sd.aux) != hipSuccess) return set_err("aux stream mark failed");
    *out = e;
    return 0;
}
static int main_wait(hipStream_t main_s, hipEvent_t e, int line = 0) {
    if (stream_wait_probed(main_s, e, line)) return set_err("stream wait failed");
    return 0;
}

enum { PANEL_ENC = 1, PANEL_DEC = 2, PANEL_VOCAB = 4, PANEL_KV = 8 };
static inline bool panel_takes(int cls, int M, int N, int K, const float* dY, int lddy, const float* X, int ldx) {
    const int mask = g_dtype == 1 ? 13 : 15;
    return (mask & cls) && gemm_wgrad_panel_takes(N, K, M, dY, lddy, X, ldx, K);
}
static inline int panel_np() { return g_dtype == 1 ? 1 : 3; }

static inline int linear_wgrad(hipStream_t s, int M, int N, int K, const float* dY, int lddy, const float* X, int ldx,
                               float* dW, float* db, int panel_cls = 0) {
    SideStream& sd = side();
    hipStream_t ws = s;
    if (sd.stream && sd.enabled) {
        TRY(side_fork(s));
        ws = sd.stream;
    }
    if (panel_cls && gemm_wgrad_panel_pending() == 0 && panel_takes(panel_cls, M, N, K, dY, lddy, X, ldx))
        return gemm_wgrad_panel(ws, panel_np(), N, K, M, dY, lddy, X, ldx, dW, K, db);
    return gemm_any(ws, 1, 0, N, K, M, dY, lddy, X, ldx, dW, K, nullptr, FIRA_GEMM_ACCUM, 0, db);
}

static inline int flush_grouped_wgrads(hipStream_t s);
static inline int group_make_room(hipStream_t s) {
    if ((g_dtype == 1 ? gemm_bf16_group_full() : gemm_group_full()) || gemm_wgrad_panel_full()) return flush_grouped_wgrads(s);
    return 0;
}
static inline int linear_wgrad_grouped(hipStream_t s, int M, int N, int K, const float* dY, int lddy, const float* X,
                                       int ldx, float* dW, float* db, int max_split = 0) {
    SideStream& sd = side();
    if (!(sd.stream && sd.enabled)) return linear_wgrad(s, M, N, K, dY, lddy, X, ldx, dW, db);
    TRY(group_make_room(s));
    if (panel_takes(PANEL_DEC, M, N, K, dY, lddy, X, ldx)) return gemm_wgrad_panel_add(N, K, M, dY, lddy, X, ldx, dW, K, db);
    if (g_dtype == 1) {
        if (!gemm_bf16_takes(N, K, M)) return linear_wgrad(s, M, N, K, dY, lddy, X, ldx, dW, db);
        return gemm_bf16_group_add_wgrad(sd.stream, N, K, M, dY, lddy, X, ldx, dW, K, db, max_split);
    }
    return gemm_group_add_wgrad(sd.stream, N, K, M, dY, lddy, X, ldx, dW, K, db, max_split);
}
static inline bool enc_group_on() {
    static const bool off = [] { const char* e = getenv("FIRA_ENC_WGRAD_GROUP"); return e && e[0] == '0'; }();
    SideStream& sd = side();
    return !off && sd.stream && sd.enabled;
}
static inline int enc_wgrad(hipStream_t s, int M, int N, int K, const float* dY, int lddy, const float* X, int ldx, float* dW,
                            float* db) {
    if (!enc_group_on()) return linear_wgrad(s, M, N, K, dY, lddy, X, ldx, dW, db, PANEL_ENC);
    SideStream& sd = side();
    TRY(group_make_room(s));
    if (panel_takes(PANEL_ENC, M, N, K, dY, lddy, X, ldx)) return gemm_wgrad_panel_add(N, K, M, dY, lddy, X, ldx, dW, K, db);
    if (g_dtype == 1) {
        if (!gemm_bf16_takes(N, K, M)) return linear_wgrad(s, M, N, K, dY, lddy, X, ldx, dW, db);
        return gemm_bf16_group_add_wgrad(sd.stream, N, K, M, dY, lddy, X, ldx, dW, K, db, 32);
    }
    return gemm_group_add_wgrad(sd.stream, N, K, M, dY, lddy, X, ldx, dW, K, db, 32);
}
static inline int wgrad_on(hipStream_t ws, int panel_cls, int M, int N, int K, const float* dY, int lddy, const float* X, int ldx,
                           float* dW, float* db) {
    if (gemm_wgrad_panel_pending() == 0 && panel_takes(panel_cls, M, N, K, dY, lddy, X, ldx))
        return gemm_wgrad_panel(ws, panel_np(), N, K, M, dY, lddy, X, ldx, dW, K, db);
    return gemm_any(ws, 1, 0, N, K, M, dY, lddy, X, ldx, dW, K, nullptr, FIRA_GEMM_ACCUM, 0, db);
}
static inline int flush_wgrad_queues(hipStream_t ws) {
    TRY(g_dtype == 1 ? gemm_bf16_group_flush(ws) : gemm_group_flush(ws));
    return gemm_wgrad_panel_flush(ws, panel_np());
}
static inline int flush_grouped_wgrads(hipStream_t s) {
    SideStream& sd = side();
    if (!(sd.stream && sd.enabled)) return 0;
    TRY(side_fork(s));
    return flush_wgrad_queues(sd.stream);
}

struct RedCollector {
    float* buf = nullptr;
    size_t cap = 0, used = 0;
    RedTable tab;
    void reset(float* b, size_t c) { buf = b; cap = c; used = 0; tab.n = 0; }
    float* alloc(size_t n, int entries = 4) {
        if (!buf || used + n > cap || tab.n + entries > RED_MAX) return nullptr;
        float* p = buf + used;
        used += (n + 63) / 64 * 64;
        return p;
    }
    void add(float* dst, const float* src, int width, int n_part, int stride) {
        tab.e[tab.n++] = RedEntry{dst, src, width, n_part, stride};
    }
};
static RedCollector& red() { static thread_local RedCollector r; return r; }

static int ln_bwd(hipStream_t s, int M, const float* dy, const float* sum, const float* stats, const float* gamma, float* ds,
                  float* dx_drop, float* dgamma, float* dbeta, float dropout, uint64_t seed, uint32_t st,
                  const int32_t* rows = nullptr,
                  const float* row_w = nullptr, float* dsum = nullptr, float* dwsum = nullptr, bool* extras = nullptr,
                  uint32_t idx0 = 0) {
    const int nb = add_layernorm_bwd_blocks(M);
    static const bool no_extra = [] { const char* e = getenv("FIRA_LN_BWD_EXTRA"); return e && e[0] == '0'; }();
    const bool want = row_w && dsum && dwsum && !no_extra;
    float* part = want ? red().alloc((size_t)nb * 4 * FIRA_D) : nullptr;
    const bool ex = part != nullptr;
    if (!part) part = red().alloc((size_t)nb * 2 * FIRA_D);
    if (extras) *extras = ex;
    const int w = ex ? 4 * FIRA_D : 2 * FIRA_D;
    TRY(add_layernorm_bwd(s, M, dy, sum, stats, gamma, ds, dx_drop, dgamma, dbeta, dropout, seed, st, rows, part,
                          ex ? row_w : nullptr, idx0));
    if (part) {
        red().add(dgamma, part, FIRA_D, nb, w);
        red().add(dbeta, part + FIRA_D, FIRA_D, nb, w);
        if (ex) {
            red().add(dsum, part + 2 * FIRA_D, FIRA_D, nb, w);
            red().add(dwsum, part + 3 * FIRA_D, FIRA_D, nb, w);
        }
    }
    return 0;
}

static int ln_bwd_dgrad(hipStream_t s, int M, int N, const float* dy, const float* sum, const float* stats, const float* gamma,
                        float* ds, float* dx_drop, float* dgamma, float* dbeta, float dropout, uint64_t seed, uint32_t st,
                        const float* W, int ldw, float* dX, int lddx, const float* relu_mask, uint32_t idx0 = 0) {
    constexpr int lnb_max_rows = 1536;
    if (g_dtype == 0 && M <= lnb_max_rows && ds != dy && gemm_tile32_takes(0, M, N, FIRA_D, dy, FIRA_D, W, ldw)) {
        const int nb = gemm_tile32_lnb_blocks(M);
        float* part = red().alloc((size_t)nb * 2 * FIRA_D);
        int rc = 0;
        if (part && gemm_tile32_lnb_try(s, M, N, dy, W, ldw, dX, lddx, relu_mask, sum, stats, gamma, ds, dx_drop, part, dropout, seed,
                                        st, &rc, idx0)) {
            TRY(rc);
            red().add(dgamma, part, FIRA_D, nb, 2 * FIRA_D);
            red().add(dbeta, part + FIRA_D, FIRA_D, nb, 2 * FIRA_D);
            return 0;
        }
    }
    TRY(ln_bwd(s, M, dy, sum, stats, gamma, ds, dx_drop, dgamma, dbeta, dropout, seed, st, nullptr, nullptr, nullptr, nullptr, nullptr, idx0));
    return gemm_any(s, 0, 0, M, N, FIRA_D, dx_drop, FIRA_D, W, ldw, dX, lddx, nullptr, 0, 0, nullptr, nullptr, relu_mask);
}

static inline int attn_bf16() { return g_dtype == 1; }

static constexpr double GCN_FUSED_MAX_DEG = 48.0;
static thread_local bool g_dense_graphs = false;
static inline bool gcn_fused_on() { return !g_dense_graphs; }
static inline void note_graph_density(const fira_batch* b) {
    g_dense_graphs = b->n_nodes > 0 && (double)b->nnz > GCN_FUSED_MAX_DEG * (double)b->n_nodes;
}


enum Site { SITE_GATE = 0, SITE_COMB_OUT = 1, SITE_GCN = 2, SITE_SELF = 3, SITE_CROSS = 4, SITE_FFN = 5 };
static inline uint32_t site(int layer, int kind) { return (uint32_t)(layer * 8 + kind + 1); }

struct Ctx {
    hipStream_t s;
    const Layout* L;
    const fira_batch* bt;
    const float* P;
    float* G;
    Plan* pl;
    float p_drop, p_gcn;
    uint64_t seed;
    int R = 0;
    const int32_t* rows = nullptr;
    int Td = 0;
    const int32_t* dec_off = nullptr;
    const int32_t* row_bt = nullptr;
    const int32_t* rows_dense = nullptr;
    bool deferred = false;
    bool kv_ragged = false;
    bool serial = false;
    float* loss_sum = nullptr;
    int32_t* n_tok = nullptr;
    hipEvent_t ev_kv[16] = {};
    int kv_waited = 0;
    hipEvent_t ev_src = nullptr;
    hipEvent_t ev_zero = nullptr;
    const fira_adam_opts* adam = nullptr;
    float* Pw = nullptr;
    bool dp_begin = false;
    bool wout_planes = false;
    bool kv_planes = false;
    int32_t* row_step = nullptr;
    fira_adam_opts rows_ad{};
    bool adam_a_only = false;
    hipEvent_t ev_early = nullptr;
    const float* count = nullptr;
    const ShadowTable* shadow_tab = nullptr;
    hipEvent_t ev_shadow = nullptr;
    int n_lanes = 1;
    struct Lane { hipStream_t s; int b0, nb, r0, nr; } lanes[2] = {};
};
typedef Ctx::Lane Lane;

static AdamRowsTables adam_rows_tables(const Layout& L, float* params, const fira_adam_opts& ad, int32_t* row_step) {
    AdamRowsTables tb;
    tb.p = params; tb.m = ad.m; tb.v = ad.v;
    tb.off[0] = L.dec_emb; tb.off[1] = L.emb;
    tb.rows[0] = tb.rows[1] = L.d.vocab;
    tb.last = row_step;
    return tb;
}

static int decoder_lanes(Ctx& c) {
    constexpr int DEC_LANES_MIN_ROWS = 768;
    static const int forced = [] { const char* e = getenv("FIRA_DEC_LANES"); return e ? (atoi(e) >= 2 ? 2 : 1) : 0; }();
    const int want = forced ? forced : (c.Td >= DEC_LANES_MIN_ROWS ? 2 : 1);
    c.n_lanes = g_lanes = 1;
    c.lanes[0] = Lane{c.s, 0, c.pl->B, 0, c.Td};
    const fira_batch& bt = *c.bt;
    if (want < 2 || !c.dec_off || !bt.dec_off_host || bt.B < 2 || !side_on() || c.serial || !c.kv_ragged) return 0;
    SideStream& sd = side();
    if (!sd.lane) {
        if (hipStreamCreateWithFlags(&sd.lane, hipStreamNonBlocking) != hipSuccess) return set_err("lane stream: create failed");
    }
    int bm = 1, best = 1 << 30;
    for (int b = 1; b < bt.B; ++b) {
        const int d = abs(2 * bt.dec_off_host[b] - c.Td);
        if (d < best) { best = d; bm = b; }
    }
    const int rm = bt.dec_off_host[bm];
    if (rm <= 0 || rm >= c.Td || bt.dec_off_host[bt.B] != c.Td) return 0;
    c.n_lanes = g_lanes = 2;
    c.lanes[0] = Lane{c.s, 0, bm, 0, rm};
    c.lanes[1] = Lane{sd.lane, bm, bt.B - bm, rm, c.Td - rm};
    return 0;
}
static int lanes_fork(Ctx& c) {
    for (int k = 1; k < c.n_lanes; ++k) {
        hipEvent_t e = side().ev();
        if (hipEventRecord(e, c.s) != hipSuccess || hipStreamWaitEvent(c.lanes[k].s, e, 0) != hipSuccess) return set_err("lane fork failed");
    }
    return 0;
}
static int lanes_join(Ctx& c) {
    for (int k = 1; k < c.n_lanes; ++k) {
        hipEvent_t e = side().ev();
        if (hipEventRecord(e, c.lanes[k].s) != hipSuccess || hipStreamWaitEvent(c.s, e, 0) != hipSuccess) return set_err("lane join failed");
    }
    return 0;
}
static int lanes_fork_to(Ctx& c, hipStream_t target) {
    for (int k = 0; k < c.n_lanes; ++k) {
        hipEvent_t e = side().ev();
        if (hipEventRecord(e, c.lanes[k].s) != hipSuccess || hipStreamWaitEvent(target, e, 0) != hipSuccess) return set_err("lane -> side stream fork failed");
    }
    return 0;
}

static inline bool fold_one_launch(int nl) { return nl <= 10; }
static inline bool comb_x3_on(int nl) { return nl <= 8; }
static inline bool gcn_x3_on(int nl) { return gcn_fused_on() && fold_one_launch(nl); }
static inline bool kv_x3_on(int nl) { return nl * 2 <= 24; }

static int adam_rows_prefetch(Ctx& c, hipStream_t st) {
// ... 374 lines not shown
    }

    float *bx = p.ddec, *by = p.dT_a, *bz = p.dT_c;
    constexpr int DEC_WGRAD_EVERY = 3;
    const int dec_every = p.nl % DEC_WGRAD_EVERY != 0 ? 0 : DEC_WGRAD_EVERY;
    {
    ProfScope prof_region(s, PROF_DEC_REGION, 0.0);
    TRY(lanes_fork(c));
    auto aux_fork_all = [&]() -> int { return c.n_lanes > 1 ? lanes_fork_to(c, side().aux) : aux_fork(s); };
    auto flush_wgrads_all = [&]() -> int {
        if (c.n_lanes == 1) return flush_grouped_wgrads(s);
        SideStream& sd = side();
        if (!(sd.stream && sd.enabled)) return 0;
        TRY(lanes_fork_to(c, sd.stream));
        return flush_wgrad_queues(sd.stream);
    };
    for (int l = p.nl - 1; l >= 0; --l) {
        ProfDecoderTag prof_tag;
        const DecLayer& w = L.dec[l];
        DecSave& e = p.dec[l];
        DecGrad& g = p.decg[l];
        const float* x_in = l == 0 ? p.x0 : p.dec[l - 1].x_f;
        hipEvent_t ev_kv_done[2] = {nullptr, nullptr};
        auto dmem_pair = [&]() -> int {
            if (!(so && (l % 2 == 0 || l == 0))) return 0;
            const int nlay = std::min(2, p.nl - l);
            const size_t o = (size_t)l * 2 * D;
            if (c.n_lanes > 1 && ev_kv_done[0] && ev_kv_done[1]) {
                for (int k = 0; k < c.n_lanes; ++k)
                    if (hipStreamWaitEvent(ss, ev_kv_done[k], 0) != hipSuccess) return set_err("lane -> auxiliary stream fork failed");
            } else
            TRY(aux_fork_all());
            prof_decoder_tag(-1);
            const int rc_kv = c.kv_planes
                    ? linear_x3_kacc(ss, Mc, p.dkv_all + o, p.kvp, p.WkvTX + (size_t)l * 2 * 3 * D * D, nlay * 2, p.dmem_c, D, true, g_dtype == 1)
                    : linear_dgrad(ss, Mc, nlay * 2 * D, D, p.dkv_all + o, p.kvp, c.P + L.wkv_all + o * D, p.dmem_c, D, true);
            prof_decoder_tag(+1);
            return rc_kv;
        };
        for (int k = 0; k < c.n_lanes; ++k) {
            const Lane& ln = c.lanes[k];
            hipStream_t ls = ln.s;
            const size_t r0 = (size_t)ln.r0;
            const int nr = ln.nr;
            const uint32_t idx0 = (uint32_t)(r0 * D);
            const int32_t* q_off = c.dec_off ? c.dec_off + ln.b0 : nullptr;
            const bool q = k == 0;
            TRY(ln_bwd_dgrad(ls, nr, p.F, bx + r0 * D, e.s_f + r0 * D, e.st_f + r0 * 2, c.P + w.lnf_g, by + r0 * D, g.dYf + r0 * D,
                             G + w.lnf_g, G + w.lnf_b, c.p_drop, c.seed, site(l, SITE_FFN), c.P + w.w2, p.F, g.dh + r0 * p.F, p.F,
                             e.h + r0 * p.F, idx0));
            if (q) TRY(linear_wgrad_grouped(s, c.Td, D, p.F, g.dYf, D, e.h, p.F, G + w.w2, G + w.b2));
            if (q) TRY(linear_wgrad_grouped(s, c.Td, p.F, D, g.dh, p.F, e.x_c, D, G + w.w1, G + w.b1));
            TRY(linear_dgrad(ls, nr, p.F, D, g.dh + r0 * p.F, p.F, c.P + w.w1, by + r0 * D, D, true));
            TRY(ln_bwd_dgrad(ls, nr, D, by + r0 * D, e.s_c + r0 * D, e.st_c + r0 * 2, c.P + w.lnc_g, bz + r0 * D, g.dYc + r0 * D,
                             G + w.lnc_g, G + w.lnc_b, c.p_drop, c.seed, site(l, SITE_CROSS), c.P + w.wo_c, D, bx + r0 * D, D, nullptr,
                             idx0));
            if (q) TRY(linear_wgrad_grouped(s, c.Td, D, D, g.dYc, D, e.ao2, D, G + w.wo_c, G + w.bo_c));
            TRY(attention_bwd(ls, ln.nb, H, p.T, Sm, e.qc, D, p.kv_all + l * 2 * D, p.kvp, p.kv_all + l * 2 * D + D, p.kvp,
                              p.mem_valid_c, 0, 0, e.ao2, D, bx, D, g.dq, D, p.dkv_all + l * 2 * D, p.kvp,
                              p.dkv_all + l * 2 * D + D, p.kvp, q_off, 0, attn_bf16(), p.mem_off + ln.b0));
            if (c.n_lanes == 1) TRY(dmem_pair());
            else if (so && l % 2 == 0 && k < 2) {
                ev_kv_done[k] = side().ev();
                if (hipEventRecord(ev_kv_done[k], ls) != hipSuccess) return set_err("lane event record failed");
            }
            if (q) TRY(linear_wgrad_grouped(s, c.Td, D, D, g.dq, D, e.x_a, D, G + w.wq_c, G + w.bq_c));
            TRY(linear_dgrad(ls, nr, D, D, g.dq + r0 * D, D, c.P + w.wq_c, bz + r0 * D, D, true));
            TRY(ln_bwd_dgrad(ls, nr, D, bz + r0 * D, e.s_a + r0 * D, e.st_a + r0 * 2, c.P + w.lns_g, by + r0 * D, g.dYs + r0 * D,
                             G + w.lns_g, G + w.lns_b, c.p_drop, c.seed, site(l, SITE_SELF), c.P + w.wo_s, D, bx + r0 * D, D, nullptr,
                             idx0));
            if (q) TRY(linear_wgrad_grouped(s, c.Td, D, D, g.dYs, D, e.ao, D, G + w.wo_s, G + w.bo_s));
            TRY(attention_bwd(ls, ln.nb, H, p.T, p.T, e.qkv, 3 * D, e.qkv + D, 3 * D, e.qkv + 2 * D, 3 * D,
                              p.tar_valid + (size_t)ln.b0 * p.T, 1, 0, e.ao, D, bx, D, g.dqkv, 3 * D, g.dqkv + D, 3 * D, g.dqkv + 2 * D,
                              3 * D, q_off, 1, attn_bf16()));
            if (q) TRY(linear_wgrad_grouped(s, c.Td, 3 * D, D, g.dqkv, 3 * D, x_in, D, G + w.wqkv, G + w.bqkv));
            TRY(linear_dgrad(ls, nr, 3 * D, D, g.dqkv + r0 * 3 * D, 3 * D, c.P + w.wqkv, by + r0 * D, D, true));
        }
        if (c.n_lanes > 1) TRY(dmem_pair());
        if (dec_every > 0 && l % dec_every == 0 && side().stream && side().enabled) {
            const int nlay = std::min(dec_every, p.nl - l);
            const size_t o = (size_t)l * 2 * D;
            prof_decoder_tag(-1);
            int rc_w = flush_wgrads_all();
            if (!rc_w)
                rc_w = wgrad_on(side().stream, PANEL_KV, Mc, nlay * 2 * D, D, p.dkv_all + o, p.kvp, p.mem_c, D, G + L.wkv_all + o * D,
                                G + L.bkv_all + o);
            prof_decoder_tag(+1);
            TRY(rc_w);
        }
        float* t = bx; bx = by; by = t;
    }
    TRY(lanes_join(c));
    }
    const float* dy = bx;
    TRY(flush_grouped_wgrads(s));
    {
        hipStream_t es = (side().stream && side().enabled) ? side().stream : s;
        if (c.row_bt) TRY(embed_rows_bwd(es, c.Td, c.row_bt, c.bt->tar, G + L.dec_emb, dy, 0));
        else TRY(embed_gather_bwd(es, p.B, p.T, c.bt->tar, G + L.dec_emb, dy, p.T, 0, 0));
    }
    hipEvent_t& ev_dmem = mid.ev_dmem;
    if (so) {
        TRY(side_mark(&ev_dmem));
    } else {
        TRY(linear_dgrad(s, Mc, KV, D, p.dkv_all, p.kvp, c.P + L.wkv_all, p.dmem_c, D, true));
    }
    if (!(side().stream && side().enabled))
        TRY(linear_wgrad(s, Mc, KV, D, p.dkv_all, p.kvp, p.mem_c, D, G + L.wkv_all, G + L.bkv_all, PANEL_KV));
    else if (dec_every == 0)
        TRY(wgrad_on(side().stream, PANEL_KV, Mc, KV, D, p.dkv_all, p.kvp, p.mem_c, D, G + L.wkv_all, G + L.bkv_all));
    TRY(deferred_reduce(side().stream && side().enabled ? side().stream : s, red().tab));
    hipEvent_t& ev_groupA = mid.ev_groupA;
    if (c.adam && side().stream && side().enabled) {
        ev_groupA = side().ev();
        if (hipEventRecord(ev_groupA, side().stream) != hipSuccess) return set_err("group-A mark failed");
    }
    if (mid_event) {
        SideStream& sd = side();
        hipStream_t es = s;
        if (sd.stream && sd.enabled) {
            TRY(aux_fork(s));
            hipEvent_t e2 = sd.ev();
            if (hipEventRecord(e2, sd.stream) != hipSuccess || hipStreamWaitEvent(sd.aux, e2, 0) != hipSuccess)
                return set_err("mid-event: weight-gradient stream mark failed");
            es = sd.aux;
        }
        hipError_t e = hipEventRecord(mid_event, es);
        if (e != hipSuccess) return set_err("hipEventRecord: %s", hipGetErrorString(e));
    }
    return 0;
}

static int backward_encoder(Ctx& c, BwdMid& mid) {
    Plan& p = *c.pl;
    const Layout& L = *c.L;
    hipStream_t s = c.s;
    const int D = FIRA_D;
    const fira_batch& bt = *c.bt;
    const int Nc = bt.n_nodes, Cc = bt.n_code, Mc = bt.n_mem;
    float* G = c.G;
    hipEvent_t ev_dmem = mid.ev_dmem, ev_groupA = mid.ev_groupA;
    float* dXn = p.dXa;
    float* other = p.dXb;
    UnfoldTable unfold_tab;
    static const bool unfold_late_off = [] { const char* e = getenv("FIRA_UNFOLD_LATE"); return e && e[0] == '0'; }();
    const bool unfold_late = !unfold_late_off && enc_group_on() && p.nl <= 16;
    const int wgrad_every = unfold_late ? enc_wgrad_every(Nc, p.nl) : 1;
    const float *uf_dW21[16], *uf_W1[16], *uf_W2[16];
    float *uf_dW1[16], *uf_dW2[16];
    int uf_n = 0;
    if (!c.ev_zero) TRY(zero(s, dXn, (size_t)Nc * D * sizeof(float)));
    if (ev_dmem) TRY(main_wait(s, ev_dmem, __LINE__));
    TRY(rows_move(s, 1, Mc, D, dXn, p.dmem_c, nullptr, bt.mem_rows));
    for (int l = p.nl - 1; l >= 0; --l) {
        const EncLayer& w = L.enc[l];
        EncSave& e = p.enc[l];
        EncGrad& g = p.encg[l];
        float* dc21 = p.dc21 + (size_t)l * D;
        bool sums = false;
        const bool room = unfold_tab.n < 16;
        TRY(ln_bwd(s, Nc, dXn, e.s2, e.st2, c.P + w.ln2g, other, g.dY2, G + w.ln2g, G + w.ln2b, c.p_gcn,
                              c.seed, site(l, SITE_GCN), nullptr, room ? p.rsum : nullptr, G + w.fc2b, dc21, &sums));
        if (sums) unfold_tab.e[unfold_tab.n++] = UnfoldEntry{c.P + w.fc2w, c.P + w.fc1b, dc21, G + w.fc2w, G + w.fc1b};
        float* dW21 = p.dW21 + (size_t)l * D * D;
        const bool grouped = enc_group_on();
        bool flushed = false;
        auto unfold = [&]() -> int {
            hipStream_t ws = s;
            if (side().stream && side().enabled) {
                if (!grouped || (!flushed && (!sums || !unfold_late))) TRY(side_fork(s));
                ws = side().stream;
            }
            if (!sums) TRY(colsum(ws, Nc, D, g.dY2, D, dc21, p.rsum));
            if (unfold_late) {
                uf_dW21[uf_n] = dW21; uf_W1[uf_n] = c.P + w.fc1w; uf_W2[uf_n] = c.P + w.fc2w;
                uf_dW1[uf_n] = G + w.fc1w; uf_dW2[uf_n] = G + w.fc2w;
                ++uf_n;
            } else {
            TRY(gemm_f32_ex(ws, 0, 1, D, D, D, dW21, D, c.P + w.fc1w, D, G + w.fc2w, D, nullptr, FIRA_GEMM_ACCUM, 0, nullptr));
            TRY(gemm_f32_ex(ws, 1, 0, D, D, D, c.P + w.fc2w, D, dW21, D, G + w.fc1w, D, nullptr, FIRA_GEMM_ACCUM, 0, nullptr));
            }
            if (!sums) TRY(gcn_bias_unfold(ws, c.P + w.fc2w, c.P + w.fc1b, dc21, G + w.fc2w, G + w.fc1b));
            return 0;
        };
        if (gcn_fused_on()) {
            TRY(gcn_fused_bwd(s, Nc, bt.rowptr, bt.col, bt.val, g.dY2, p.W21 + (size_t)l * D * D, e.Z, other, g_dtype == 1,
                              gcn_x3_on(p.nl) ? p.W21tx + (size_t)l * 3 * D * D : nullptr));
            TRY(enc_wgrad(s, Nc, D, D, e.Z, D, p.X[l], D, dW21, nullptr));
            if (!sums) TRY(colsum(s, Nc, D, g.dY2, D, G + w.fc2b));
            if (!grouped) TRY(unfold());
        } else {
        TRY(enc_wgrad(s, Nc, D, D, g.dY2, D, e.Z, D, dW21, sums ? nullptr : G + w.fc2b));
        if (!grouped) TRY(unfold());
        TRY(linear_dgrad(s, Nc, D, D, g.dY2, D, p.W21 + (size_t)l * D * D, p.dNB2, D, false));
        TRY(csr_spmm_ex(s, Nc, bt.rowptr, bt.col, bt.val, p.dNB2, D, other, D, 0, 1, 1, nullptr));
        }
        const int nb_comb = comb_fused_bwd_parts();
        float* part_ln = red().alloc((size_t)nb_comb * 6 * D, 6);
        const bool comb_done = part_ln != nullptr;
        if (comb_done) {
            float* part_v = part_ln + (size_t)nb_comb * 2 * D;
            TRY(comb_fused_bwd(s, Cc, other, bt.code_rows, e.s1, e.st1, c.P + w.ln1g, c.P + w.wo, c.P + w.wqk, e.qk,
                               p.vtab_all + l * D, p.nl * D, bt.code_mark, g.dYc, g.dqk, part_ln, part_v, c.p_drop, c.seed,
                               site(l, SITE_GATE), site(l, SITE_COMB_OUT), g_dtype == 1,
                               comb_x3_on(p.nl) ? p.WcTX + (size_t)l * 9 * D * D : nullptr));
            red().add(G + w.ln1g, part_ln, D, nb_comb, 2 * D);
            red().add(G + w.ln1b, part_ln + D, D, nb_comb, 2 * D);
            for (int k = 0; k < 4; ++k)
                red().add(p.dvtab_all + (size_t)k * p.nl * D + l * D, part_v + k * D, D, nb_comb, 4 * D);
            TRY(enc_wgrad(s, Cc, D, D, g.dYc, D, e.c, D, G + w.wo, G + w.bo));
        } else {
        TRY(ln_bwd(s, Cc, other, e.s1, e.st1, c.P + w.ln1g, other, g.dYc, G + w.ln1g, G + w.ln1b, c.p_drop,
                              c.seed, site(l, SITE_COMB_OUT), bt.code_rows));
        TRY(enc_wgrad(s, Cc, D, D, g.dYc, D, e.c, D, G + w.wo, G + w.bo));
        TRY(linear_dgrad(s, Cc, D, D, g.dYc, D, c.P + w.wo, p.dCB_a, D, false));
        {
            const int nb = combination_bwd_blocks(Cc);
            float* part = red().alloc((size_t)nb * 4 * D);
            TRY(combination_bwd(s, Cc, e.qk, p.vtab_all + l * D, p.nl * D, bt.code_mark, p.dCB_a, g.dqk,
                                p.dvtab_all + l * D, p.nl * D, c.p_drop, c.seed, site(l, SITE_GATE), part));
            if (part)
                for (int k = 0; k < 4; ++k)
                    red().add(p.dvtab_all + (size_t)k * p.nl * D + l * D, part + k * D, D, nb, 4 * D);
        }
        }
        TRY(enc_wgrad(s, Cc, 2 * D, D, g.dqk, 2 * D, e.Xc, D, G + w.wqk, G + w.bqk));
        if (grouped) {
            if ((p.nl - l) % wgrad_every == 0 || l == 0) { TRY(flush_grouped_wgrads(s)); flushed = true; }
            TRY(unfold());
        }
        if (!comb_done)
            TRY(gemm_any(s, 0, 0, Cc, D, 2 * D, g.dqk, 2 * D, c.P + w.wqk, D, other, D, nullptr, FIRA_GEMM_ACCUM, 0, nullptr,
                         bt.code_rows));
        float* tmp = dXn; dXn = other; other = tmp;
    }
    if (uf_n > 0) TRY(gcn_unfold_products(side().stream, uf_n, uf_dW21, uf_W1, uf_W2, uf_dW1, uf_dW2));
    hipEvent_t ev_tail = nullptr;
    int64_t adam_b0 = L.split;
    {
        const bool ax = side_on();
        hipStream_t rs = ax ? side().aux : s;
        if (ax) TRY(aux_fork(s));
        TRY(deferred_reduce(rs, red().tab));
        TRY(gemm_f32_ex(rs, 1, 0, p.nl * D, D, 4, p.dvtab_all, p.nl * D, c.P + L.mark_emb, D, G + L.w2_all, D, nullptr,
                        FIRA_GEMM_ACCUM, 1, G + L.b2_all));
        TRY(gemm_f32_ex(rs, 0, 0, 3, D, p.nl * D, p.dvtab_all + (size_t)p.nl * D, p.nl * D, c.P + L.w2_all, D, G + L.mark_emb + D, D,
                        nullptr, FIRA_GEMM_ACCUM, std::max(2, p.nl), nullptr));
        if (ax) TRY(side_mark(&ev_tail));
    }
    if (bt.emb_item_tok && bt.emb_item_ptr && bt.emb_rows && bt.ast_rows && bt.ast_ids && L.d.ast_vocab <= 128) {
        TRY(embed_grouped_bwd(s, bt.n_emb_items, bt.emb_item_tok, bt.emb_item_ptr, bt.emb_rows, G + L.emb, dXn));
        TRY(embed_list_bwd_small(s, bt.n_ast_items, bt.ast_rows, bt.ast_ids, G + L.ast_emb, dXn, L.d.ast_vocab));
    } else {
        TRY(zero(s, p.H, (size_t)p.NB * D * sizeof(float)));
        TRY(rows_move(s, 1, Nc, D, p.H, dXn, nullptr, bt.node_rows));
        TRY(embed_gather_bwd(s, p.B, p.L, bt.sou, G + L.emb, p.H, p.N, 0, 0));
        TRY(embed_gather_bwd(s, p.B, p.S, bt.sub_token, G + L.emb, p.H, p.N, p.L, 0));
        if (L.d.ast_vocab <= 128)
            TRY(embed_gather_bwd_small(s, p.B, p.A, bt.ast_change, G + L.ast_emb, p.H, p.N, p.L + p.S, 0, L.d.ast_vocab));
        else
            TRY(embed_gather_bwd(s, p.B, p.A, bt.ast_change, G + L.ast_emb, p.H, p.N, p.L + p.S, 0));
    }
    if (c.adam) {
        const fira_adam_opts& ad = *c.adam;
        if (c.adam_a_only) {
            if (c.ev_early) TRY(main_wait(s, c.ev_early, __LINE__));
            const int64_t a0 = c.row_step ? L.dec_emb + (int64_t)L.d.vocab * D : 0;
            if (c.count) TRY(adam_step(s, L.split - a0, c.Pw + a0, G + a0, ad.m + a0, ad.v + a0, ad.lr, ad.beta1, ad.beta2, ad.eps, ad.step, c.count, 1));
            else TRY(adam_step_mb(s, L.split - a0, c.Pw + a0, G + a0, nullptr, ad.m + a0, ad.v + a0, ad.lr, ad.beta1, ad.beta2, ad.eps, ad.step, c.n_tok, nullptr));
            if (c.row_step)
                TRY(adam_rows_step(s, adam_rows_tables(L, c.Pw, ad, c.row_step), G, ad.lr, ad.beta1, ad.beta2, ad.eps, ad.step,
                                   c.count ? nullptr : c.n_tok, c.count, 1));
        } else {
        if (ev_groupA) TRY(main_wait(s, ev_groupA, __LINE__));
        const int64_t a0 = c.row_step ? L.dec_emb + (int64_t)L.d.vocab * D : 0;
        TRY(adam_step_mb(s, L.split - a0, c.Pw + a0, G + a0, nullptr, ad.m + a0, ad.v + a0, ad.lr, ad.beta1, ad.beta2, ad.eps,
                         ad.step, c.n_tok, nullptr));
        }
        if (!c.adam_a_only) adam_b0 = L.mark_emb;
        if (c.row_step && !c.adam_a_only) {
            TRY(adam_rows_step(s, adam_rows_tables(L, c.Pw, ad, c.row_step), G, ad.lr, ad.beta1, ad.beta2, ad.eps, ad.step,
                               c.n_tok, nullptr));
            adam_b0 = L.ast_emb;
        } else
        if (adam_b0 > L.split)
        TRY(adam_step_mb(s, adam_b0 - L.split, c.Pw + L.split, G + L.split, nullptr, ad.m + L.split, ad.v + L.split, ad.lr, ad.beta1,
                         ad.beta2, ad.eps, ad.step, c.n_tok, nullptr));
    }
    if (ev_tail) TRY(main_wait(s, ev_tail, __LINE__));
    if (side().stream && side().enabled) TRY(side_join(s, __LINE__));
    TRY(gcn_bias_unfold_all(s, unfold_tab));
    if (c.adam && !c.adam_a_only) {
        const fira_adam_opts& ad = *c.adam;
        TRY(adam_step_mb(s, L.live - adam_b0, c.Pw + adam_b0, G + adam_b0, nullptr, ad.m + adam_b0, ad.v + adam_b0, ad.lr, ad.beta1,
                         ad.beta2, ad.eps, ad.step, c.n_tok, nullptr));
    }
    return 0;
}

static int backward(Ctx& c, int R, const int32_t* rows, hipEvent_t mid_event) {
    BwdMid mid;
    TRY(backward_decoder(c, R, rows, mid_event, mid));
    return backward_encoder(c, mid);
}

static int check_batch(const fira_batch* b) {
    FIRA_REQUIRE(b && b->B > 0, "empty batch");
    FIRA_REQUIRE(b->sou && b->mark && b->ast_change && b->sub_token && b->rowptr && b->col && b->val,
                 "batch has null encoder inputs");
    FIRA_REQUIRE(b->node_rows && b->code_rows && b->code_mark && b->mem_rows && b->mem_dst,
                 "batch has null node lists (node_rows / code_rows / code_mark / mem_rows / mem_dst)");
    FIRA_REQUIRE(b->n_nodes > 0 && b->n_code > 0 && b->n_mem > 0 && b->n_code <= b->n_nodes && b->n_mem <= b->n_nodes,
                 "inconsistent node counts %d / %d / %d", b->n_nodes, b->n_code, b->n_mem);
    note_graph_density(b);
    return 0;
}
static int check_counts(const fira_batch* b, const Plan& p) {
    FIRA_REQUIRE(b->n_nodes <= p.NB && b->n_code <= p.CB && b->n_mem <= p.MB, "node lists exceed the batch geometry");
    return 0;
}

struct DecodePlan {
    Plan enc;
    int BR;
    float *kc[2], *vc[2];
    int32_t* hist[2];
    float *x, *q, *qkv, *ao, *s, *xa, *qc, *xc, *h, *tgt, *score, *gate, *logits;
    float* wsT;
    uint16_t* kv16;
    size_t build(void* ws, const fira_dims& d, int B, int n_beam, int flags = 0) {
        size_t used = enc.build(ws, d, B, false);
        Arena a(ws ? (char*)ws + used : nullptr);
        BR = B * n_beam;
        const size_t D = FIRA_D, T = d.tar_len, cache = (size_t)d.n_layer * BR * T * D;
        for (int i = 0; i < 2; ++i) {
            kc[i] = a.f(cache); vc[i] = a.f(cache);
            hist[i] = a.get<int32_t>((size_t)BR * T);
        }
        x = a.f(BR * D); q = a.f(BR * D); qkv = a.f(BR * 3 * D); ao = a.f(BR * D); s = a.f(BR * D); xa = a.f(BR * D); qc = a.f(BR * D);
        xc = a.f(BR * D); h = a.f((size_t)BR * d.d_ff); tgt = a.f(BR * D);
        score = a.f((size_t)BR * (d.sou_len + d.sub_len)); gate = a.f((size_t)BR * 2);
        logits = a.f((size_t)BR * enc.ldl);
        wsT = a.f((size_t)d.n_layer * 2 * D * D);
        kv16 = (flags & FIRA_DECODE_KV_BF16) ? a.get<uint16_t>((size_t)enc.MB * enc.kvp) : nullptr;
        return used + a.used;
    }
};

}

using namespace fira;

extern "C" {

size_t fira_workspace_bytes(const fira_dims* d, int B, int mode) {
    if (!get_layout(d) || B <= 0) return 0;
    Plan p;
    return p.build(nullptr, *d, B, mode == 1);
}
size_t fira_decode_workspace_bytes(const fira_dims* d, int B, int n_beam) {
    return fira_decode_workspace_bytes_ex(d, B, n_beam, 0);
}
size_t fira_decode_workspace_bytes_ex(const fira_dims* d, int B, int n_beam, int flags) {
    if (!get_layout(d) || B <= 0 || n_beam <= 0 || (flags & ~FIRA_DECODE_KV_BF16)) return 0;
    DecodePlan dp;
    return dp.build(nullptr, *d, B, n_beam, flags);
}

struct PendingStep {
    bool active = false;
    Plan plan;
    fira_batch batch;
    Ctx ctx{};
    BwdMid mid;
    int dtype = 0;
    const float* params = nullptr;
    const ShadowTable* tab = nullptr;
    const float* W21 = nullptr;
    int64_t W21n = 0;
    const uint16_t *W21b = nullptr, *W21bT = nullptr;
};
static thread_local PendingStep g_pending;

static int train_call(void* stream, const fira_dims* d, const fira_batch* batch, const float* params, float* grads,
                      void* workspace, size_t workspace_bytes, const fira_train_opts* opts, float* loss_sum,
                      int32_t* n_tok, void* mid_event, float* params_w, const fira_adam_opts* adam, bool begin_only = false,
                      int32_t* row_step = nullptr) {
// ... 442 lines not shown
```

fira_icse_amd/csrc/gcn_fused.hip:

```cpp
#include "engine.h"
#include "mfma_frag.h"
#include "epilogue.h"
#include "x3.h"

namespace fira {

constexpr int GF_TILE = 16;
constexpr int GF_TMAX = 4;
constexpr int GF_ROWS = GF_TILE * GF_TMAX;
constexpr int GF_WAVES = 16;
constexpr int GF_RPW = GF_ROWS / GF_WAVES;
constexpr int GF_GRID = 256;
constexpr size_t GF_LDS = 84 * 1024;
constexpr size_t GX_PLANE = (size_t)GF_ROWS * 512;
constexpr size_t GF_LDS_X3 = 3 * GX_PLANE + 1024;

typedef float f32x4acc __attribute__((ext_vector_type(4)));

struct GcnFusedArgs {
    int n_rows;
    const int32_t *rowptr, *col;
    const float* val;
    const float* X;
    const float* W;
    const float *bias, *r1_col, *res, *gamma, *beta;
    float *sum, *y, *stats, *rowsum_out;
    const int32_t* slot2;
    float* y2;
    float p, inv_keep;
    uint64_t seed;
    uint32_t site;
    float* u_out;
    float* acc_out;
};

__device__ __forceinline__ int gf_off(int row, int quad) { return row * FIRA_D + ((quad ^ (row & 11)) << 2); }

template <bool BF, bool BWD, int NP = 0>
__global__ __launch_bounds__(GF_WAVES * 64) void gcn_fused_kernel(const GcnFusedArgs a) {
    constexpr bool X3 = NP > 0;
    extern __shared__ __attribute__((aligned(16))) float gf_lds[];
    float* const sm_u = gf_lds;
    char* const sm_p = reinterpret_cast<char*>(gf_lds);
    float* const sm_rs = X3 ? gf_lds + 3 * GX_PLANE / 4 : gf_lds + GF_ROWS * FIRA_D;
    const int t = threadIdx.x, lane = t & 63, wave = t >> 6;
    const int l15 = lane & 15, kq = lane >> 4;
    const int wg = (blockIdx.x & 7) * (GF_GRID / 8) + (blockIdx.x >> 3);
    const int n_tiles = (a.n_rows + GF_TILE - 1) / GF_TILE;
    const int tq = n_tiles / GF_GRID, tr = n_tiles % GF_GRID;
    const int t_beg = wg * tq + min(wg, tr), t_cnt = tq + (wg < tr ? 1 : 0);
    int a_off[4], d_off[4], r_off[GF_RPW];
#pragma unroll
    for (int ii = 0; ii < 4; ++ii) a_off[ii] = gf_off(l15, kq * 4 + ii);
#pragma unroll
    for (int r = 0; r < 4; ++r) d_off[r] = gf_off(4 * kq + r, (wave * 16 + l15) >> 2) + (l15 & 3);
#pragma unroll
    for (int i = 0; i < GF_RPW; ++i) r_off[i] = gf_off(wave * GF_RPW + i, lane);

    for (int pass = 0; pass < t_cnt; pass += GF_TMAX) {
        const int nt = min(GF_TMAX, t_cnt - pass);
        const int row0 = (t_beg + pass) * GF_TILE;
        const int row_end = min(a.n_rows, row0 + nt * GF_TILE);
        if (wave * GF_RPW < nt * GF_TILE) {
            const int rbase = row0 + wave * GF_RPW;
            int rp = 0;
            if (lane <= GF_RPW) rp = a.rowptr[min(rbase + lane, a.n_rows)];
            int beg[GF_RPW], cnt[GF_RPW];
#pragma unroll
            for (int i = 0; i < GF_RPW; ++i) {
                beg[i] = __builtin_amdgcn_readlane(rp, i);
                cnt[i] = rbase + i < row_end ? __builtin_amdgcn_readlane(rp, i + 1) - beg[i] : 0;
            }
            const int gi = lane >> 4, ge = lane & 15;
            const int my_beg = __shfl(rp, gi, 64);
            const int my_cnt = rbase + gi < row_end ? __shfl(rp, gi + 1, 64) - my_beg : 0;
            int c = 0;
            float v = 0.f;
            if (ge < my_cnt) {
                c = a.col[my_beg + ge];
                v = a.val[my_beg + ge];
            }
            int cmax = 0;
#pragma unroll
            for (int i = 0; i < GF_RPW; ++i) cmax = max(cmax, min(cnt[i], 16));
            f32x4v acc[GF_RPW];
#pragma unroll
            for (int i = 0; i < GF_RPW; ++i) acc[i] = f32x4v{0.f, 0.f, 0.f, 0.f};
            for (int jb = 0; jb < cmax; jb += 4) {
                f32x4v x[GF_RPW][4];
                float w[GF_RPW][4];
#pragma unroll
                for (int i = 0; i < GF_RPW; ++i)
#pragma unroll
                    for (int u = 0; u < 4; ++u) {
                        const int src = i * 16 + jb + u;
                        const int cj = __builtin_amdgcn_readlane(c, src);
                        w[i][u] = __builtin_bit_cast(float, __builtin_amdgcn_readlane(__builtin_bit_cast(int, v), src));
                        x[i][u] = *reinterpret_cast<const f32x4v*>(a.X + (size_t)cj * FIRA_D + lane * 4);
                    }
#pragma unroll
                for (int i = 0; i < GF_RPW; ++i)
#pragma unroll
                    for (int u = 0; u < 4; ++u) {
                        acc[i].x = fmaf(w[i][u], x[i][u].x, acc[i].x); acc[i].y = fmaf(w[i][u], x[i][u].y, acc[i].y);
                        acc[i].z = fmaf(w[i][u], x[i][u].z, acc[i].z); acc[i].w = fmaf(w[i][u], x[i][u].w, acc[i].w);
                    }
            }
            float vs = v;
            vs = sum16(vs);
            float vsum[GF_RPW];
#pragma unroll
            for (int i = 0; i < GF_RPW; ++i) vsum[i] = __builtin_bit_cast(float, __builtin_amdgcn_readlane(__builtin_bit_cast(int, vs), i * 16));
#pragma unroll
            for (int i = 0; i < GF_RPW; ++i) {
                if (cnt[i] <= 16) continue;
                float extra = 0.f;
                for (int base = beg[i] + 16; base < beg[i] + cnt[i]; base += 64) {
                    const int n = min(64, beg[i] + cnt[i] - base);
                    int c2 = 0;
                    float v2 = 0.f;
                    if (lane < n) {
                        c2 = a.col[base + lane];
                        v2 = a.val[base + lane];
                    }
                    extra += v2;
                    for (int j = 0; j < n; j += 4) {
                        f32x4v x4[4];
                        float w4[4];
#pragma unroll
                        for (int u = 0; u < 4; ++u) {
                            const int sl = min(j + u, 63);
                            const int cj = j + u < 64 ? __builtin_amdgcn_readlane(c2, sl) : 0;
                            w4[u] = j + u < 64 ? __builtin_bit_cast(float, __builtin_amdgcn_readlane(__builtin_bit_cast(int, v2), sl)) : 0.f;
                            x4[u] = *reinterpret_cast<const f32x4v*>(a.X + (size_t)cj * FIRA_D + lane * 4);
                        }
#pragma unroll
                        for (int u = 0; u < 4; ++u) {
                            acc[i].x = fmaf(w4[u], x4[u].x, acc[i].x); acc[i].y = fmaf(w4[u], x4[u].y, acc[i].y);
                            acc[i].z = fmaf(w4[u], x4[u].z, acc[i].z); acc[i].w = fmaf(w4[u], x4[u].w, acc[i].w);
                        }
                    }
                }
                extra = wave_sum(extra);
                vsum[i] += extra;
            }
#pragma unroll
            for (int i = 0; i < GF_RPW; ++i) {
                const int lr = wave * GF_RPW + i;
                if constexpr (X3) {
                    gx_store_row4<X3 ? NP : 3>(sm_p, GX_PLANE, lr, lane, acc[i]);
                } else
                *reinterpret_cast<f32x4v*>(&sm_u[r_off[i]]) = acc[i];
                if (lane == 0) sm_rs[lr] = vsum[i];
                if (BWD && rbase + i < row_end && a.u_out)
                    *reinterpret_cast<f32x4v*>(a.u_out + (size_t)(rbase + i) * FIRA_D + lane * 4) = acc[i];
                if (!BWD && a.rowsum_out && lane == 0 && rbase + i < row_end) a.rowsum_out[rbase + i] = vsum[i];
            }
        }
        const rsrc_t rW = buf_rsrc(a.W, X3 ? 3u * (unsigned)GX_WPLANE : FIRA_D * FIRA_D * 4u);
        const unsigned wlane = (unsigned)((kq * 16) * FIRA_D + wave * 16 + l15) * 4u;
        float b[2][16];
        const unsigned xlane = gx_wlane(wave, lane);
        uint4 bx[2][3];
        if constexpr (X3) {
#pragma unroll
            for (int pl = 0; pl < NP; ++pl)
                bx[0][pl] = __builtin_bit_cast(uint4, __builtin_amdgcn_raw_buffer_load_b128(rW, xlane, pl * (int)GX_WPLANE, 0));
        } else {
#pragma unroll
        for (int s2 = 0; s2 < 16; ++s2)
            b[0][s2] = __builtin_bit_cast(float, __builtin_amdgcn_raw_buffer_load_b32(rW, wlane, s2 * FIRA_D * 4, 0));
        }
        asm volatile("" ::: "memory");
        lds_barrier();   

        f32x4acc acc[GF_TMAX];
#pragma unroll
        for (int tt = 0; tt < GF_TMAX; ++tt) acc[tt] = f32x4acc{0.f, 0.f, 0.f, 0.f};
        if constexpr (X3) {
            const int a_q = gx_frag_base(l15, kq);
#pragma unroll
            for (int ks = 0; ks < 8; ++ks) {
                if (ks + 1 < 8) {
#pragma unroll
                    for (int pl = 0; pl < NP; ++pl)
                        bx[(ks + 1) & 1][pl] = __builtin_bit_cast(uint4, __builtin_amdgcn_raw_buffer_load_b128(
                                                                              rW, xlane, pl * (int)GX_WPLANE + (ks + 1) * 1024, 0));
                }
                asm volatile("" ::: "memory");
#pragma unroll
                for (int tt = 0; tt < GF_TMAX; ++tt) {
                    if (tt < nt)
                        gx_terms<X3 ? NP : 3>(acc[tt], sm_p + ((a_q ^ (ks << 6)) + tt * (GF_TILE * 512)), GX_PLANE, bx[ks & 1]);
                }
                asm volatile("" ::: "memory");
            }
        } else {
            constexpr int NC = FIRA_D / 64;
#pragma unroll
            for (int c = 0; c < NC; ++c) {
                if (c + 1 < NC) {
#pragma unroll
                    for (int s2 = 0; s2 < 16; ++s2)
                        b[(c + 1) & 1][s2] = __builtin_bit_cast(float, __builtin_amdgcn_raw_buffer_load_b32(
                                                                           rW, wlane, ((c + 1) * 64 + s2) * FIRA_D * 4, 0));
                }
                asm volatile("" ::: "memory");
#pragma unroll
                for (int tt = 0; tt < GF_TMAX; ++tt) {
                    if (tt < nt) {
                        float af[16];
#pragma unroll
                        for (int ii = 0; ii < 4; ++ii) {
                            const f32x4v q = *reinterpret_cast<const f32x4v*>(&sm_u[a_off[ii] + tt * (GF_TILE * FIRA_D) + c * 64]);
                            af[4 * ii] = q.x; af[4 * ii + 1] = q.y; af[4 * ii + 2] = q.z; af[4 * ii + 3] = q.w;
                        }
                        if constexpr (BF) {
#pragma unroll
                            for (int j = 0; j < 2; ++j) {
                                uint4 ua, ub;
                                ua.x = apk2(af[8 * j], af[8 * j + 1]); ua.y = apk2(af[8 * j + 2], af[8 * j + 3]);
                                ua.z = apk2(af[8 * j + 4], af[8 * j + 5]); ua.w = apk2(af[8 * j + 6], af[8 * j + 7]);
                                ub.x = apk2(b[c & 1][8 * j], b[c & 1][8 * j + 1]); ub.y = apk2(b[c & 1][8 * j + 2], b[c & 1][8 * j + 3]);
                                ub.z = apk2(b[c & 1][8 * j + 4], b[c & 1][8 * j + 5]); ub.w = apk2(b[c & 1][8 * j + 6], b[c & 1][8 * j + 7]);
                                acc[tt] = __builtin_amdgcn_mfma_f32_16x16x32_bf16(__builtin_bit_cast(abf16x8, ua),
                                                                                  __builtin_bit_cast(abf16x8, ub), acc[tt], 0, 0, 0);
                            }
                        } else {
#pragma unroll
                            for (int s2 = 0; s2 < 16; ++s2)
                                acc[tt] = __builtin_amdgcn_mfma_f32_16x16x4f32(af[s2], b[c & 1][s2], acc[tt], 0, 0, 0);
                        }
                    }
                }
                asm volatile("" ::: "memory");
            }
        }
        lds_barrier();
#pragma unroll
        for (int tt = 0; tt < GF_TMAX; ++tt) {
            if (tt < nt) {
#pragma unroll
                for (int r = 0; r < 4; ++r) sm_u[d_off[r] + tt * (GF_TILE * FIRA_D)] = acc[tt][r];
            }
        }
        lds_barrier();   

        const int rbase = row0 + wave * GF_RPW;
        if (rbase < row_end) {
            if constexpr (BWD) {
                f32x4v old[GF_RPW];
#pragma unroll
                for (int i = 0; i < GF_RPW; ++i) {
                    const int row = min(rbase + i, row_end - 1);
                    old[i] = *reinterpret_cast<const f32x4v*>(a.acc_out + (size_t)row * FIRA_D + lane * 4);
                }
#pragma unroll
                for (int i = 0; i < GF_RPW; ++i) {
                    if (rbase + i >= row_end) continue;
                    const f32x4v d = *reinterpret_cast<const f32x4v*>(&sm_u[r_off[i]]);
                    *reinterpret_cast<f32x4v*>(a.acc_out + (size_t)(rbase + i) * FIRA_D + lane * 4) = old[i] + d;
                }
            } else {
                const f32x4v bias4 = *reinterpret_cast<const f32x4v*>(a.bias + lane * 4);
                const f32x4v c4 = *reinterpret_cast<const f32x4v*>(a.r1_col + lane * 4);
                const f32x4v g4 = *reinterpret_cast<const f32x4v*>(a.gamma + lane * 4);
                const f32x4v be4 = *reinterpret_cast<const f32x4v*>(a.beta + lane * 4);
                f32x4v res[GF_RPW];
                int s2[GF_RPW];
#pragma unroll
                for (int i = 0; i < GF_RPW; ++i) {
                    const int row = min(rbase + i, row_end - 1);
                    res[i] = *reinterpret_cast<const f32x4v*>(a.res + (size_t)row * FIRA_D + lane * 4);
                    s2[i] = a.slot2 ? a.slot2[row] : -1;
                }
#pragma unroll
                for (int i = 0; i < GF_RPW; ++i) {
                    const int row = rbase + i;
                    if (row >= row_end) continue;
                    const int lr = wave * GF_RPW + i;
                    f32x4v x = *reinterpret_cast<const f32x4v*>(&sm_u[r_off[i]]);
                    x = x + bias4;
                    const float w = sm_rs[lr];
                    x.x = fmaf(w, c4.x, x.x); x.y = fmaf(w, c4.y, x.y); x.z = fmaf(w, c4.z, x.z); x.w = fmaf(w, c4.w, x.w);
                    if (a.p > 0.f) {
                        const uint32_t e0 = (uint32_t)row * FIRA_D + lane * 4;
                        x.x *= dropout_scale(a.seed, a.site, e0 + 0, a.p, a.inv_keep);
                        x.y *= dropout_scale(a.seed, a.site, e0 + 1, a.p, a.inv_keep);
                        x.z *= dropout_scale(a.seed, a.site, e0 + 2, a.p, a.inv_keep);
                        x.w *= dropout_scale(a.seed, a.site, e0 + 3, a.p, a.inv_keep);
                    }
                    x = x + res[i];
                    const float mean = wave_sum(x.x + x.y + x.z + x.w) * (1.0f / FIRA_D);
                    const f32x4v d = x - mean;
                    const float var = wave_sum(d.x * d.x + d.y * d.y + d.z * d.z + d.w * d.w) * (1.0f / FIRA_D);
                    const float rstd = 1.0f / sqrtf(var + 1e-5f);
                    const size_t o = (size_t)row * FIRA_D + lane * 4;
                    __builtin_nontemporal_store(x, reinterpret_cast<f32x4v*>(a.sum + o));
                    const f32x4v out = {d.x * rstd * g4.x + be4.x, d.y * rstd * g4.y + be4.y, d.z * rstd * g4.z + be4.z,
                                        d.w * rstd * g4.w + be4.w};
                    *reinterpret_cast<f32x4v*>(a.y + o) = out;
                    if (s2[i] >= 0) *reinterpret_cast<f32x4v*>(a.y2 + (size_t)s2[i] * FIRA_D + lane * 4) = out;
                    if (lane == 0) {
                        a.stats[2 * row] = mean;
                        a.stats[2 * row + 1] = rstd;
                    }
                }
            }
        }
        if (pass + GF_TMAX < t_cnt) lds_barrier();
    }
}

static double gcn_fused_bytes(int n_rows, bool bwd) {
    return 4.0 * (n_rows + 1) + (bwd ? 4.0 : 3.0) * n_rows * FIRA_D * 4.0;
}
template <typename K>
static int gcn_fused_lds(K kernel, size_t bytes = GF_LDS) {
    const hipError_t e = hipFuncSetAttribute((const void*)kernel, hipFuncAttributeMaxDynamicSharedMemorySize, (int)bytes);
    return e == hipSuccess ? 0 : set_err("gcn_fused: cannot raise the dynamic LDS limit: %s", hipGetErrorString(e));
}

int gcn_fused_fwd(hipStream_t s, int n_rows, const int32_t* rowptr, const int32_t* col, const float* val, const float* X,
                  const float* Wk, const float* bias, const float* r1_col, const float* gamma, const float* beta, float* sum,
                  float* y, float* stats, float* rowsum_out, const int32_t* slot2, float* y2, float dropout, uint64_t seed,
                  uint32_t site, int bf16, const uint16_t* Wx) {
    if (n_rows <= 0) return 0;
    FIRA_REQUIRE(rowptr && col && val && X && Wk && bias && r1_col && gamma && beta && sum && y && stats,
                 "gcn_fused_fwd: null pointer argument");
    FIRA_REQUIRE((uintptr_t)X % 16 == 0 && (uintptr_t)Wk % 16 == 0 && (uintptr_t)sum % 16 == 0 && (uintptr_t)y % 16 == 0,
                 "gcn_fused_fwd: rows must be 16-byte aligned");
    ProfScope prof(s, PROF_GCN, 2.0 * n_rows * FIRA_D * FIRA_D, gcn_fused_bytes(n_rows, false));
    GcnFusedArgs a{};
    a.n_rows = n_rows; a.rowptr = rowptr; a.col = col; a.val = val; a.X = X; a.W = Wk;
    a.bias = bias; a.r1_col = r1_col; a.res = X; a.gamma = gamma; a.beta = beta;
    a.sum = sum; a.y = y; a.stats = stats; a.rowsum_out = rowsum_out; a.slot2 = y2 ? slot2 : nullptr; a.y2 = y2;
    a.p = dropout; a.inv_keep = dropout > 0.f ? 1.0f / (1.0f - dropout) : 1.0f; a.seed = seed; a.site = site;
    static const int attr = gcn_fused_lds(gcn_fused_kernel<true, false>) | gcn_fused_lds(gcn_fused_kernel<false, false>) |
                            gcn_fused_lds(gcn_fused_kernel<false, false, 3>, GF_LDS_X3) |
                            gcn_fused_lds(gcn_fused_kernel<false, false, 1>, GF_LDS_X3);
    if (attr) return attr;
    if (Wx) {
        a.W = reinterpret_cast<const float*>(Wx);
        if (bf16) hipLaunchKernelGGL((gcn_fused_kernel<false, false, 1>), dim3(GF_GRID), dim3(GF_WAVES * 64), GF_LDS_X3, s, a);
        else hipLaunchKernelGGL((gcn_fused_kernel<false, false, 3>), dim3(GF_GRID), dim3(GF_WAVES * 64), GF_LDS_X3, s, a);
    } else
    if (bf16) hipLaunchKernelGGL((gcn_fused_kernel<true, false>), dim3(GF_GRID), dim3(GF_WAVES * 64), GF_LDS, s, a);
    else hipLaunchKernelGGL((gcn_fused_kernel<false, false>), dim3(GF_GRID), dim3(GF_WAVES * 64), GF_LDS, s, a);
    FIRA_CHECK_LAUNCH("gcn_fused_fwd");
    return 0;
}

int gcn_fused_bwd(hipStream_t s, int n_rows, const int32_t* rowptr, const int32_t* col, const float* val, const float* dY,
                  const float* Wk, float* u_out, float* acc_out, int bf16, const uint16_t* Wx) {
    if (n_rows <= 0) return 0;
    FIRA_REQUIRE(rowptr && col && val && dY && Wk && acc_out, "gcn_fused_bwd: null pointer argument");
    FIRA_REQUIRE((uintptr_t)dY % 16 == 0 && (uintptr_t)Wk % 16 == 0 && (uintptr_t)acc_out % 16 == 0 && (uintptr_t)u_out % 16 == 0,
                 "gcn_fused_bwd: rows must be 16-byte aligned");
    ProfScope prof(s, PROF_GCN, 2.0 * n_rows * FIRA_D * FIRA_D, gcn_fused_bytes(n_rows, true));
    GcnFusedArgs a{};
    a.n_rows = n_rows; a.rowptr = rowptr; a.col = col; a.val = val; a.X = dY; a.W = Wk;
    a.u_out = u_out; a.acc_out = acc_out;
    static const int attr = gcn_fused_lds(gcn_fused_kernel<true, true>) | gcn_fused_lds(gcn_fused_kernel<false, true>) |
                            gcn_fused_lds(gcn_fused_kernel<false, true, 3>, GF_LDS_X3) |
                            gcn_fused_lds(gcn_fused_kernel<false, true, 1>, GF_LDS_X3);
    if (attr) return attr;
    if (Wx) {
        a.W = reinterpret_cast<const float*>(Wx);
        if (bf16) hipLaunchKernelGGL((gcn_fused_kernel<false, true, 1>), dim3(GF_GRID), dim3(GF_WAVES * 64), GF_LDS_X3, s, a);
        else hipLaunchKernelGGL((gcn_fused_kernel<false, true, 3>), dim3(GF_GRID), dim3(GF_WAVES * 64), GF_LDS_X3, s, a);
    } else
    if (bf16) hipLaunchKernelGGL((gcn_fused_kernel<true, true>), dim3(GF_GRID), dim3(GF_WAVES * 64), GF_LDS, s, a);
    else hipLaunchKernelGGL((gcn_fused_kernel<false, true>), dim3(GF_GRID), dim3(GF_WAVES * 64), GF_LDS, s, a);
    FIRA_CHECK_LAUNCH("gcn_fused_bwd");
    return 0;
}

struct SplitTable { int n = 0; const float* src[48]; uint16_t* dst[48]; };
__global__ __launch_bounds__(256) void gcn_split_planes_kernel(const SplitTable tab) {
    const int m = blockIdx.y, j = blockIdx.x * 256 + threadIdx.x;
    const int n = j >> 5, c = j & 31;
    const float* src = tab.src[m] + (size_t)n * FIRA_D + c * 8;
    f32x4v u0 = *reinterpret_cast<const f32x4v*>(src), u1 = *reinterpret_cast<const f32x4v*>(src + 4);
    const int unit = ((n >> 4) * 8 + (c >> 2)) * 64 + (c & 3) * 16 + (n & 15);
    uint16_t* dst = tab.dst[m] + (size_t)unit * 8;
#pragma unroll
    for (int pl = 0; pl < 3; ++pl) {
        const uint32_t p0 = gx_pack(u0.x, u0.y), p1 = gx_pack(u0.z, u0.w), p2 = gx_pack(u1.x, u1.y), p3 = gx_pack(u1.z, u1.w);
        *reinterpret_cast<uint4*>(dst + (size_t)pl * FIRA_D * FIRA_D) = uint4{p0, p1, p2, p3};
        if (pl < 2) {
            u0.x = gx_rest_lo(u0.x, p0); u0.y = gx_rest_hi(u0.y, p0); u0.z = gx_rest_lo(u0.z, p1); u0.w = gx_rest_hi(u0.w, p1);
            u1.x = gx_rest_lo(u1.x, p2); u1.y = gx_rest_hi(u1.y, p2); u1.z = gx_rest_lo(u1.z, p3); u1.w = gx_rest_hi(u1.w, p3);
        }
    }
}
int gcn_split_planes(hipStream_t s, int n, const float* const* src, uint16_t* const* dst) {
    if (n <= 0) return 0;
    FIRA_REQUIRE(n <= 48, "gcn_split_planes: %d matrices", n);
    SplitTable tab;
    tab.n = n;
    for (int i = 0; i < n; ++i) { tab.src[i] = src[i]; tab.dst[i] = dst[i]; }
    hipLaunchKernelGGL(gcn_split_planes_kernel, dim3(FIRA_D * FIRA_D / 8 / 256, n), dim3(256), 0, s, tab);
    FIRA_CHECK_LAUNCH("gcn_split_planes");
    return 0;
}

__global__ __launch_bounds__(256) void transpose256_kernel(const float* __restrict__ W, float* __restrict__ Wt) {
    __shared__ float tile[64][65];
    const int l = blockIdx.z, r0 = blockIdx.y * 64, c0 = blockIdx.x * 64;
    const float* src = W + (size_t)l * FIRA_D * FIRA_D;
    float* dst = Wt + (size_t)l * FIRA_D * FIRA_D;
    const int tx = threadIdx.x & 63, ty = threadIdx.x >> 6;
    for (int r = ty; r < 64; r += 4) tile[r][tx] = src[(size_t)(r0 + r) * FIRA_D + c0 + tx];
    __syncthreads();
    for (int r = ty; r < 64; r += 4) dst[(size_t)(c0 + r) * FIRA_D + r0 + tx] = tile[tx][r];
}
int transpose256(hipStream_t s, int nl, const float* W, float* Wt) {
    if (nl <= 0) return 0;
    hipLaunchKernelGGL(transpose256_kernel, dim3(FIRA_D / 64, FIRA_D / 64, nl), dim3(256), 0, s, W, Wt);
    FIRA_CHECK_LAUNCH("transpose256");
    return 0;
}

}

extern "C" {
int fira_gcn_layer_fwd(void* stream, int n_rows, const int32_t* rowptr, const int32_t* col, const float* val, const float* X,
                       const float* W21t, const float* bias, const float* c21, const float* gamma, const float* beta,
                       float* sum, float* y, float* stats, float* rowsum_out, float dropout, uint64_t seed, uint32_t site,
                       int dtype) {
    FIRA_REQUIRE(dtype >= FIRA_F32 && dtype <= FIRA_BF16X1, "fira_gcn_layer_fwd: dtype must be FIRA_F32, FIRA_BF16, FIRA_F32X3 or FIRA_BF16X1");
    return fira::gcn_fused_fwd((hipStream_t)stream, n_rows, rowptr, col, val, X, W21t, bias, c21, gamma, beta, sum, y, stats,
                               rowsum_out, nullptr, nullptr, dropout, seed, site, dtype == FIRA_BF16 || dtype == FIRA_BF16X1,
                               dtype >= FIRA_F32X3 ? reinterpret_cast<const uint16_t*>(W21t) : nullptr);
}
int fira_gcn_layer_bwd(void* stream, int n_rows, const int32_t* rowptr, const int32_t* col, const float* val, const float* dY,
                       const float* W21, float* V, float* dX, int dtype) {
    FIRA_REQUIRE(dtype >= FIRA_F32 && dtype <= FIRA_BF16X1, "fira_gcn_layer_bwd: dtype must be FIRA_F32, FIRA_BF16, FIRA_F32X3 or FIRA_BF16X1");
    FIRA_REQUIRE(V != nullptr, "fira_gcn_layer_bwd: V (the weight gradient's operand) must be given");
    return fira::gcn_fused_bwd((hipStream_t)stream, n_rows, rowptr, col, val, dY, W21, V, dX, dtype == FIRA_BF16 || dtype == FIRA_BF16X1,
                               dtype >= FIRA_F32X3 ? reinterpret_cast<const uint16_t*>(W21) : nullptr);
}
int fira_gcn_weight_planes(void* stream, int n_mats, const float* B, uint16_t* planes) {
    FIRA_REQUIRE(B && planes && n_mats > 0 && n_mats <= 24, "fira_gcn_weight_planes: bad argument");
    FIRA_REQUIRE((uintptr_t)B % 16 == 0 && (uintptr_t)planes % 16 == 0, "fira_gcn_weight_planes: 16-byte aligned pointers");
    const float* src[24];
    uint16_t* dst[24];
    for (int i = 0; i < n_mats; ++i) { src[i] = B + (size_t)i * FIRA_D * FIRA_D; dst[i] = planes + (size_t)i * 3 * FIRA_D * FIRA_D; }
    return fira::gcn_split_planes((hipStream_t)stream, n_mats, src, dst);
}
}
```

Measured before the change: 13890 commits/s.

## Fold next layer's LayerNorm backward into GCN and combine backward epilogues

For encoder layers above the first, the LayerNorm backward of the layer below is now computed inside the epilogues of the fused GCN and combine backward kernels. The kernels write ds and the dropout-masked dx directly and park per-block column partial sums for gamma, beta, fc2 bias and the row-weighted sum. The standalone ln_bwd launch and its extra read of the gradient are skipped for those layers. In exchange the kernels need more LDS and extra barriers, and the reduction partial buffers grow.

After: 13790 commits/s, median of 2. About the same (-0.8%).

```diff
diff --git a/fira_icse_amd/build.py b/fira_icse_amd/build.py
--- a/fira_icse_amd/build.py
+++ b/fira_icse_amd/build.py
@@ -9,7 +9,7 @@
 CSRC = os.path.join(HERE, "csrc")
 LIB = os.path.join(HERE, "libfira_hip.so")
 SOURCES = ["gemm_f32.hip", "gemm_bf16.hip", "gemm_wgrad_panel.hip", "gemm_bf16_panel.hip", "gemm_small.hip", "spmm.hip", "spmm_dense.hip", "gcn_fused.hip", "comb_fused.hip", "head_x3.hip", "rowops.hip", "attention.hip", "copyhead.hip", "beam.hip", "engine.hip", "layout.cpp", "hostlists.cpp"]
-HEADERS = ["common.h", "engine.h", "epilogue.h", "mfma_frag.h", "x3.h", os.path.join("..", "..", "include", "fira_hip.h")]
+HEADERS = ["common.h", "engine.h", "epilogue.h", "ln_fold.h", "mfma_frag.h", "x3.h", os.path.join("..", "..", "include", "fira_hip.h")]
 FLAGS = ["--offload-arch=gfx950", "-O3", "-std=c++17", "-fPIC", "-munsafe-fp-atomics", "-Wno-unused-result"]
 
 
diff --git a/fira_icse_amd/csrc/comb_fused.hip b/fira_icse_amd/csrc/comb_fused.hip
--- a/fira_icse_amd/csrc/comb_fused.hip
+++ b/fira_icse_amd/csrc/comb_fused.hip
@@ -2,6 +2,7 @@
 #include "mfma_frag.h"
 #include "epilogue.h"
 #include "x3.h"
+#include "ln_fold.h"
 
 namespace fira {
 
@@ -651,11 +652,13 @@
     float p, inv_keep;
     uint64_t seed;
     uint32_t site_gate, site_out;
+    LnBwdFold ln;
 };
 
 constexpr size_t CBX_PLANE = (size_t)CB_ROWS * 512;
-constexpr size_t CB_LDS_X3 = 100 * 1024;
-constexpr size_t CB_LDS_X3_2 = 2 * 3 * (size_t)2 * CF_TILE * 512 + 256 + 48 * 1024 + 1024;
+constexpr size_t CB_LDS_X3 = 104 * 1024;
+constexpr size_t CB_LDS_X3_2 = 2 * 3 * (size_t)2 * CF_TILE * 512 + 256 + 52 * 1024 + 1024;
+constexpr size_t CB_LDS = 88 * 1024;
 template <bool BF, int NP = 0, int TM = 1>
 __global__ __launch_bounds__(CF_WAVES * 64) void comb_fused_bwd_kernel(const CombFusedBwdArgs a) {
     constexpr int CB_TMAX = TM, CB_ROWS = CF_TILE * TM, CB_RPW = CB_ROWS / CF_WAVES;
@@ -697,6 +700,10 @@
     *reinterpret_cast<f32x4v*>(&red[wave * 2 * FIRA_D + FIRA_D + lane * 4]) = f32x4v{0.f, 0.f, 0.f, 0.f};
 #pragma unroll
     for (int m = 0; m < 4; ++m) redv[(kq * 4 + m) * FIRA_D + col] = 0.f;
+    const bool fold = a.ln.ds != nullptr;
+    constexpr int FCOLS = (2 * (int)PANEL - CB_ROWS * FIRA_D) / 16 < 1024 ? (2 * (int)PANEL - CB_ROWS * FIRA_D) / 16 : 1024;
+    float* const fold_acc = redv + 4 * 4 * FIRA_D;
+    fold_acc[t] = 0.f;
 
     for (int pass = 0; pass < t_cnt; pass += CB_TMAX) {
         const int nt = min(CB_TMAX, t_cnt - pass);
@@ -827,6 +834,26 @@
             }
         }
         lds_barrier();   
+        if (fold) {
+            const f32x4v gam = *reinterpret_cast<const f32x4v*>(a.ln.gamma + lane * 4);
+            f32x4v fsv[CB_RPW];
+            float fmean[CB_RPW], frstd[CB_RPW], frw[CB_RPW];
+#pragma unroll
+            for (int i = 0; i < CB_RPW; ++i) {
+                fsv[i] = *reinterpret_cast<const f32x4v*>(a.ln.sum + (size_t)nr[i] * FIRA_D + lane * 4);
+                fmean[i] = a.ln.stats[2 * nr[i]];
+                frstd[i] = a.ln.stats[2 * nr[i] + 1];
+                frw[i] = a.ln.row_w[nr[i]];
+            }
+            f32x4v cs[4] = {};
+#pragma unroll
+            for (int i = 0; i < CB_RPW; ++i) {
+                if (rbase + i >= row_end) continue;
+                const f32x4v x = *reinterpret_cast<const f32x4v*>(&sm_u[r_off[i]]);
+                ln_fold_row(a.ln, nr[i], lane, ds[i] + x, fsv[i], fmean[i], frstd[i], frw[i], gam, cs);
+            }
+            ln_fold_park<FCOLS>(sm_u + CB_ROWS * FIRA_D, cs, fold_acc, wave, lane, t);
+        } else
 #pragma unroll
         for (int i = 0; i < CB_RPW; ++i) {
             if (rbase + i >= row_end) continue;
@@ -847,14 +874,17 @@
         a.part_v[(size_t)blockIdx.x * 4 * FIRA_D + t] = (redv[(0 * 4 + m) * FIRA_D + cc] + redv[(1 * 4 + m) * FIRA_D + cc]) +
                                                         (redv[(2 * 4 + m) * FIRA_D + cc] + redv[(3 * 4 + m) * FIRA_D + cc]);
     }
+    if (fold) ln_fold_store(a.ln, fold_acc, t);
 }
 
 int comb_fused_bwd_parts() { return CF_GRID; }
 int comb_fused_bwd(hipStream_t s, int n_rows, float* dG, const int32_t* rows, const float* sum, const float* stats,
                    const float* gamma, const float* Wo, const float* Wqk, const float* qk, const float* vtab, int ldv,
                    const int32_t* mark, float* dYc, float* dqk, float* part_ln, float* part_v, float dropout, uint64_t seed,
-                   uint32_t site_gate, uint32_t site_out, int bf16, const uint16_t* WTx) {
+                   uint32_t site_gate, uint32_t site_out, int bf16, const uint16_t* WTx, const LnBwdFold* fold) {
     if (n_rows <= 0) return 0;
+    FIRA_REQUIRE(!fold || (fold->sum && fold->stats && fold->gamma && fold->row_w && fold->ds && fold->dx && fold->part &&
+                           fold->ds != dG), "comb_fused_bwd: incomplete LayerNorm fold");
     FIRA_REQUIRE(dG && rows && sum && stats && gamma && Wo && Wqk && qk && vtab && mark && dYc && dqk && part_ln && part_v,
                  "comb_fused_bwd: null pointer argument");
     FIRA_REQUIRE((uintptr_t)dG % 16 == 0 && (uintptr_t)sum % 16 == 0 && (uintptr_t)dYc % 16 == 0 && (uintptr_t)Wo % 16 == 0,
@@ -866,10 +896,11 @@
     a.vtab = vtab; a.ldv = ldv; a.mark = mark; a.dYc = dYc; a.dqk = dqk; a.part_ln = part_ln; a.part_v = part_v;
     a.p = dropout; a.inv_keep = dropout > 0.f ? 1.0f / (1.0f - dropout) : 1.0f; a.seed = seed; a.site_gate = site_gate;
     a.site_out = site_out;
+    if (fold) a.ln = *fold;
     static const int attr = [] {
-        hipError_t e = hipFuncSetAttribute((const void*)comb_fused_bwd_kernel<false>, hipFuncAttributeMaxDynamicSharedMemorySize, (int)CF_LDS);
+        hipError_t e = hipFuncSetAttribute((const void*)comb_fused_bwd_kernel<false>, hipFuncAttributeMaxDynamicSharedMemorySize, (int)CB_LDS);
         if (e == hipSuccess)
-            e = hipFuncSetAttribute((const void*)comb_fused_bwd_kernel<true>, hipFuncAttributeMaxDynamicSharedMemorySize, (int)CF_LDS);
+            e = hipFuncSetAttribute((const void*)comb_fused_bwd_kernel<true>, hipFuncAttributeMaxDynamicSharedMemorySize, (int)CB_LDS);
         if (e == hipSuccess)
             e = hipFuncSetAttribute((const void*)comb_fused_bwd_kernel<false, 3>, hipFuncAttributeMaxDynamicSharedMemorySize, (int)CB_LDS_X3);
         if (e == hipSuccess)
@@ -891,8 +922,8 @@
         if (bf16) hipLaunchKernelGGL((comb_fused_bwd_kernel<false, 1>), dim3(CF_GRID), dim3(CF_WAVES * 64), CB_LDS_X3, s, a);
         else hipLaunchKernelGGL((comb_fused_bwd_kernel<false, 3>), dim3(CF_GRID), dim3(CF_WAVES * 64), CB_LDS_X3, s, a);
     } else
-    if (bf16) hipLaunchKernelGGL(comb_fused_bwd_kernel<true>, dim3(CF_GRID), dim3(CF_WAVES * 64), CF_LDS, s, a);
-    else hipLaunchKernelGGL(comb_fused_bwd_kernel<false>, dim3(CF_GRID), dim3(CF_WAVES * 64), CF_LDS, s, a);
+    if (bf16) hipLaunchKernelGGL(comb_fused_bwd_kernel<true>, dim3(CF_GRID), dim3(CF_WAVES * 64), CB_LDS, s, a);
+    else hipLaunchKernelGGL(comb_fused_bwd_kernel<false>, dim3(CF_GRID), dim3(CF_WAVES * 64), CB_LDS, s, a);
     FIRA_CHECK_LAUNCH("comb_fused_bwd");
     return 0;
 }
diff --git a/fira_icse_amd/csrc/engine.h b/fira_icse_amd/csrc/engine.h
--- a/fira_icse_amd/csrc/engine.h
+++ b/fira_icse_amd/csrc/engine.h
@@ -69,8 +69,18 @@
                   const float* Wk, const float* bias, const float* r1_col, const float* gamma, const float* beta, float* sum,
                   float* y, float* stats, float* rowsum_out, const int32_t* slot2, float* y2, float dropout, uint64_t seed,
                   uint32_t site, int bf16, const uint16_t* Wx = nullptr);
+struct LnBwdFold {
+    const float *sum = nullptr, *stats = nullptr, *gamma = nullptr, *row_w = nullptr;
+    float *ds = nullptr, *dx = nullptr, *part = nullptr;
+    const int32_t* code_slot = nullptr;
+    float p = 0.f, inv_keep = 1.f;
+    uint64_t seed = 0;
+    uint32_t site = 0;
+};
 int gcn_fused_bwd(hipStream_t s, int n_rows, const int32_t* rowptr, const int32_t* col, const float* val, const float* dY,
-                  const float* Wk, float* u_out, float* acc_out, int bf16, const uint16_t* Wx = nullptr);
+                  const float* Wk, float* u_out, float* acc_out, int bf16, const uint16_t* Wx = nullptr,
+                  const LnBwdFold* fold = nullptr);
+int gcn_fused_bwd_parts();
 int gcn_split_planes(hipStream_t s, int n, const float* const* src, uint16_t* const* dst);
 size_t head_logits_x3_scratch_elems(int R);
 int head_logits_x3(hipStream_t s, int R, int V, const float* x, int ldx, const float* W, const float* bias, float* out, int ldo,
@@ -90,7 +100,8 @@
 int comb_fused_bwd(hipStream_t s, int n_rows, float* dG, const int32_t* rows, const float* sum, const float* stats,
                    const float* gamma, const float* Wo, const float* Wqk, const float* qk, const float* vtab, int ldv,
                    const int32_t* mark, float* dYc, float* dqk, float* part_ln, float* part_v, float dropout, uint64_t seed,
-                   uint32_t site_gate, uint32_t site_out, int bf16, const uint16_t* WTx = nullptr);
+                   uint32_t site_gate, uint32_t site_out, int bf16, const uint16_t* WTx = nullptr,
+                   const LnBwdFold* fold = nullptr);
 struct TransposeTable { int n = 0; const float* src[24]; float* dst[24]; };
 int transpose256_table(hipStream_t s, const TransposeTable& tab);
 int embed_gather_fwd(hipStream_t s, int B, int L, const int32_t* idx, const float* table, const float* pos, float* out,
diff --git a/fira_icse_amd/csrc/engine.hip b/fira_icse_amd/csrc/engine.hip
--- a/fira_icse_amd/csrc/engine.hip
+++ b/fira_icse_amd/csrc/engine.hip
@@ -146,7 +146,8 @@
         if (training) {
             dXa = a.f((size_t)NB * D); dXb = a.f((size_t)NB * D); dNB2 = a.f((size_t)NB * D);
             dCB_a = a.f((size_t)CB * D);
-            red_cap = (size_t)nl * ((size_t)cdiv(NB, 16) * 4 * D + (size_t)cdiv(CB, 16) * 2 * D)
+            red_cap = (size_t)nl * ((size_t)std::max(cdiv(NB, 16), gcn_fused_bwd_parts() + comb_fused_bwd_parts()) * 4 * D
+                                    + (size_t)cdiv(CB, 16) * 2 * D)
                     + (size_t)3 * nl * cdiv(TB, 16) * 2 * D
                     + (size_t)nl * std::max((size_t)cdiv(CB, 16) * 4 * D, (size_t)comb_fused_bwd_parts() * 6 * D + 64)
                     + (size_t)cdiv(L + S, 16) * B * COPY_PART_STRIDE + 4096;
@@ -525,14 +526,17 @@
 };
 static RedCollector& red() { static thread_local RedCollector r; return r; }
 
+static bool ln_bwd_extra_on() {
+    static const bool no_extra = [] { const char* e = getenv("FIRA_LN_BWD_EXTRA"); return e && e[0] == '0'; }();
+    return !no_extra;
+}
 static int ln_bwd(hipStream_t s, int M, const float* dy, const float* sum, const float* stats, const float* gamma, float* ds,
                   float* dx_drop, float* dgamma, float* dbeta, float dropout, uint64_t seed, uint32_t st,
                   const int32_t* rows = nullptr,
                   const float* row_w = nullptr, float* dsum = nullptr, float* dwsum = nullptr, bool* extras = nullptr,
                   uint32_t idx0 = 0) {
     const int nb = add_layernorm_bwd_blocks(M);
-    static const bool no_extra = [] { const char* e = getenv("FIRA_LN_BWD_EXTRA"); return e && e[0] == '0'; }();
-    const bool want = row_w && dsum && dwsum && !no_extra;
+    const bool want = row_w && dsum && dwsum && ln_bwd_extra_on();
     float* part = want ? red().alloc((size_t)nb * 4 * FIRA_D) : nullptr;
     const bool ex = part != nullptr;
     if (!part) part = red().alloc((size_t)nb * 2 * FIRA_D);
@@ -1213,16 +1217,40 @@
     if (!c.ev_zero) TRY(zero(s, dXn, (size_t)Nc * D * sizeof(float)));
     if (ev_dmem) TRY(main_wait(s, ev_dmem, __LINE__));
     TRY(rows_move(s, 1, Mc, D, dXn, p.dmem_c, nullptr, bt.mem_rows));
+    bool folded_in = false;
     for (int l = p.nl - 1; l >= 0; --l) {
         const EncLayer& w = L.enc[l];
         EncSave& e = p.enc[l];
         EncGrad& g = p.encg[l];
         float* dc21 = p.dc21 + (size_t)l * D;
-        bool sums = false;
+        bool sums = folded_in;
         const bool room = unfold_tab.n < 16;
-        TRY(ln_bwd(s, Nc, dXn, e.s2, e.st2, c.P + w.ln2g, other, g.dY2, G + w.ln2g, G + w.ln2b, c.p_gcn,
-                              c.seed, site(l, SITE_GCN), nullptr, room ? p.rsum : nullptr, G + w.fc2b, dc21, &sums));
+        if (!folded_in)
+            TRY(ln_bwd(s, Nc, dXn, e.s2, e.st2, c.P + w.ln2g, other, g.dY2, G + w.ln2g, G + w.ln2b, c.p_gcn,
+                                  c.seed, site(l, SITE_GCN), nullptr, room ? p.rsum : nullptr, G + w.fc2b, dc21, &sums));
         if (sums) unfold_tab.e[unfold_tab.n++] = UnfoldEntry{c.P + w.fc2w, c.P + w.fc1b, dc21, G + w.fc2w, G + w.fc1b};
+        const int nb_comb = comb_fused_bwd_parts();
+        float* part_ln = red().alloc((size_t)nb_comb * 6 * D, 6);
+        const bool comb_done = part_ln != nullptr;
+        LnBwdFold fold;
+        float* fold_part = nullptr;
+        if (l > 0 && gcn_fused_on() && comb_done && ln_bwd_extra_on() && unfold_tab.n < 16)
+            fold_part = red().alloc((size_t)(gcn_fused_bwd_parts() + nb_comb) * 4 * D, 4);
+        if (fold_part) {
+            const EncLayer& wb = L.enc[l - 1];
+            float* dc21b = p.dc21 + (size_t)(l - 1) * D;
+            fold.sum = p.enc[l - 1].s2; fold.stats = p.enc[l - 1].st2; fold.gamma = c.P + wb.ln2g; fold.row_w = p.rsum;
+            fold.ds = dXn; fold.dx = p.encg[l - 1].dY2; fold.part = fold_part; fold.code_slot = p.code_slot;
+            fold.p = c.p_gcn; fold.inv_keep = c.p_gcn > 0.f ? 1.0f / (1.0f - c.p_gcn) : 1.0f; fold.seed = c.seed;
+            fold.site = site(l - 1, SITE_GCN);
+            const int np = gcn_fused_bwd_parts() + nb_comb;
+            red().add(G + wb.ln2g, fold_part, D, np, 4 * D);
+            red().add(G + wb.ln2b, fold_part + D, D, np, 4 * D);
+            red().add(G + wb.fc2b, fold_part + 2 * D, D, np, 4 * D);
+            red().add(dc21b, fold_part + 3 * D, D, np, 4 * D);
+        }
+        LnBwdFold fold_comb = fold;
+        if (fold_part) fold_comb.part = fold_part + (size_t)gcn_fused_bwd_parts() * 4 * D;
         float* dW21 = p.dW21 + (size_t)l * D * D;
         const bool grouped = enc_group_on();
         bool flushed = false;
@@ -1246,7 +1274,7 @@
         };
         if (gcn_fused_on()) {
             TRY(gcn_fused_bwd(s, Nc, bt.rowptr, bt.col, bt.val, g.dY2, p.W21 + (size_t)l * D * D, e.Z, other, g_dtype == 1,
-                              gcn_x3_on(p.nl) ? p.W21tx + (size_t)l * 3 * D * D : nullptr));
+                              gcn_x3_on(p.nl) ? p.W21tx + (size_t)l * 3 * D * D : nullptr, fold_part ? &fold : nullptr));
             TRY(enc_wgrad(s, Nc, D, D, e.Z, D, p.X[l], D, dW21, nullptr));
             if (!sums) TRY(colsum(s, Nc, D, g.dY2, D, G + w.fc2b));
             if (!grouped) TRY(unfold());
@@ -1256,15 +1284,12 @@
         TRY(linear_dgrad(s, Nc, D, D, g.dY2, D, p.W21 + (size_t)l * D * D, p.dNB2, D, false));
         TRY(csr_spmm_ex(s, Nc, bt.rowptr, bt.col, bt.val, p.dNB2, D, other, D, 0, 1, 1, nullptr));
         }
-        const int nb_comb = comb_fused_bwd_parts();
-        float* part_ln = red().alloc((size_t)nb_comb * 6 * D, 6);
-        const bool comb_done = part_ln != nullptr;
         if (comb_done) {
             float* part_v = part_ln + (size_t)nb_comb * 2 * D;
             TRY(comb_fused_bwd(s, Cc, other, bt.code_rows, e.s1, e.st1, c.P + w.ln1g, c.P + w.wo, c.P + w.wqk, e.qk,
                                p.vtab_all + l * D, p.nl * D, bt.code_mark, g.dYc, g.dqk, part_ln, part_v, c.p_drop, c.seed,
                                site(l, SITE_GATE), site(l, SITE_COMB_OUT), g_dtype == 1,
-                               comb_x3_on(p.nl) ? p.WcTX + (size_t)l * 9 * D * D : nullptr));
+                               comb_x3_on(p.nl) ? p.WcTX + (size_t)l * 9 * D * D : nullptr, fold_part ? &fold_comb : nullptr));
             red().add(G + w.ln1g, part_ln, D, nb_comb, 2 * D);
             red().add(G + w.ln1b, part_ln + D, D, nb_comb, 2 * D);
             for (int k = 0; k < 4; ++k)
@@ -1294,6 +1319,7 @@
             TRY(gemm_any(s, 0, 0, Cc, D, 2 * D, g.dqk, 2 * D, c.P + w.wqk, D, other, D, nullptr, FIRA_GEMM_ACCUM, 0, nullptr,
                          bt.code_rows));
         float* tmp = dXn; dXn = other; other = tmp;
+        folded_in = fold_part != nullptr;
     }
     if (uf_n > 0) TRY(gcn_unfold_products(side().stream, uf_n, uf_dW21, uf_W1, uf_W2, uf_dW1, uf_dW2));
     hipEvent_t ev_tail = nullptr;
diff --git a/fira_icse_amd/csrc/gcn_fused.hip b/fira_icse_amd/csrc/gcn_fused.hip
--- a/fira_icse_amd/csrc/gcn_fused.hip
+++ b/fira_icse_amd/csrc/gcn_fused.hip
@@ -2,6 +2,7 @@
 #include "mfma_frag.h"
 #include "epilogue.h"
 #include "x3.h"
+#include "ln_fold.h"
 
 namespace fira {
 
@@ -13,7 +14,7 @@
 constexpr int GF_GRID = 256;
 constexpr size_t GF_LDS = 84 * 1024;
 constexpr size_t GX_PLANE = (size_t)GF_ROWS * 512;
-constexpr size_t GF_LDS_X3 = 3 * GX_PLANE + 1024;
+constexpr size_t GF_LDS_X3 = 3 * GX_PLANE + 1024 + 4096;
 
 typedef float f32x4acc __attribute__((ext_vector_type(4)));
 
@@ -32,6 +33,7 @@
     uint32_t site;
     float* u_out;
     float* acc_out;
+    LnBwdFold ln;
 };
 
 __device__ __forceinline__ int gf_off(int row, int quad) { return row * FIRA_D + ((quad ^ (row & 11)) << 2); }
@@ -57,6 +59,9 @@
 #pragma unroll
     for (int i = 0; i < GF_RPW; ++i) r_off[i] = gf_off(wave * GF_RPW + i, lane);
 
+    const bool fold = BWD && a.ln.ds != nullptr;
+    float* const fold_acc = sm_rs + 256;
+    if (fold) fold_acc[t] = 0.f;
     for (int pass = 0; pass < t_cnt; pass += GF_TMAX) {
         const int nt = min(GF_TMAX, t_cnt - pass);
         const int row0 = (t_beg + pass) * GF_TILE;
@@ -247,6 +252,7 @@
         lds_barrier();   
 
         const int rbase = row0 + wave * GF_RPW;
+        f32x4v cs[4] = {};
         if (rbase < row_end) {
             if constexpr (BWD) {
                 f32x4v old[GF_RPW];
@@ -255,6 +261,30 @@
                     const int row = min(rbase + i, row_end - 1);
                     old[i] = *reinterpret_cast<const f32x4v*>(a.acc_out + (size_t)row * FIRA_D + lane * 4);
                 }
+                if (fold) {
+                    f32x4v sv[GF_RPW];
+                    float mean[GF_RPW], rstd[GF_RPW], rw[GF_RPW];
+                    int code[GF_RPW];
+                    const f32x4v gam = *reinterpret_cast<const f32x4v*>(a.ln.gamma + lane * 4);
+#pragma unroll
+                    for (int i = 0; i < GF_RPW; ++i) {
+                        const int row = min(rbase + i, row_end - 1);
+                        sv[i] = *reinterpret_cast<const f32x4v*>(a.ln.sum + (size_t)row * FIRA_D + lane * 4);
+                        mean[i] = a.ln.stats[2 * row];
+                        rstd[i] = a.ln.stats[2 * row + 1];
+                        rw[i] = a.ln.row_w[row];
+                        code[i] = a.ln.code_slot[row];
+                    }
+#pragma unroll
+                    for (int i = 0; i < GF_RPW; ++i) {
+                        if (rbase + i >= row_end) continue;
+                        const f32x4v d = *reinterpret_cast<const f32x4v*>(&sm_u[r_off[i]]);
+                        if (code[i] >= 0)
+                            *reinterpret_cast<f32x4v*>(a.acc_out + (size_t)(rbase + i) * FIRA_D + lane * 4) = old[i] + d;
+                        else
+                            ln_fold_row(a.ln, rbase + i, lane, old[i] + d, sv[i], mean[i], rstd[i], rw[i], gam, cs);
+                    }
+                } else
 #pragma unroll
                 for (int i = 0; i < GF_RPW; ++i) {
                     if (rbase + i >= row_end) continue;
@@ -308,8 +338,10 @@
                 }
             }
         }
+        if (BWD && fold) ln_fold_park<1024>(sm_u, cs, fold_acc, wave, lane, t);
         if (pass + GF_TMAX < t_cnt) lds_barrier();
     }
+    if (BWD && fold) ln_fold_store(a.ln, fold_acc, t);
 }
 
 static double gcn_fused_bytes(int n_rows, bool bwd) {
@@ -351,9 +383,12 @@
     return 0;
 }
 
+int gcn_fused_bwd_parts() { return GF_GRID; }
 int gcn_fused_bwd(hipStream_t s, int n_rows, const int32_t* rowptr, const int32_t* col, const float* val, const float* dY,
-                  const float* Wk, float* u_out, float* acc_out, int bf16, const uint16_t* Wx) {
+                  const float* Wk, float* u_out, float* acc_out, int bf16, const uint16_t* Wx, const LnBwdFold* fold) {
     if (n_rows <= 0) return 0;
+    FIRA_REQUIRE(!fold || (fold->sum && fold->stats && fold->gamma && fold->row_w && fold->ds && fold->dx && fold->part &&
+                           fold->code_slot && fold->ds != acc_out), "gcn_fused_bwd: incomplete LayerNorm fold");
     FIRA_REQUIRE(rowptr && col && val && dY && Wk && acc_out, "gcn_fused_bwd: null pointer argument");
     FIRA_REQUIRE((uintptr_t)dY % 16 == 0 && (uintptr_t)Wk % 16 == 0 && (uintptr_t)acc_out % 16 == 0 && (uintptr_t)u_out % 16 == 0,
                  "gcn_fused_bwd: rows must be 16-byte aligned");
@@ -361,6 +396,7 @@
     GcnFusedArgs a{};
     a.n_rows = n_rows; a.rowptr = rowptr; a.col = col; a.val = val; a.X = dY; a.W = Wk;
     a.u_out = u_out; a.acc_out = acc_out;
+    if (fold) a.ln = *fold;
     static const int attr = gcn_fused_lds(gcn_fused_kernel<true, true>) | gcn_fused_lds(gcn_fused_kernel<false, true>) |
                             gcn_fused_lds(gcn_fused_kernel<false, true, 3>, GF_LDS_X3) |
                             gcn_fused_lds(gcn_fused_kernel<false, true, 1>, GF_LDS_X3);
diff --git a/fira_icse_amd/csrc/ln_fold.h b/fira_icse_amd/csrc/ln_fold.h
--- /dev/null
+++ b/fira_icse_amd/csrc/ln_fold.h
@@ -0,0 +1,56 @@
+#pragma once
+#include <hip/hip_runtime.h>
+#include <stdint.h>
+#include "common.h"
+#include "engine.h"
+#include "mfma_frag.h"
+
+namespace fira {
+
+__device__ __forceinline__ void ln_fold_row(const LnBwdFold& f, int row, int lane, f32x4v dy, f32x4v sv, float mean, float rstd,
+                                            float rw, f32x4v gam, f32x4v (&cs)[4]) {
+    const f32x4v xh = (sv - mean) * rstd;
+    cs[0] += dy * xh;
+    cs[1] += dy;
+    const f32x4v h = dy * gam;
+    const f32x4v hx = h * xh;
+    const float m1 = wave_sum(h.x + h.y + h.z + h.w) * (1.0f / FIRA_D);
+    const float m2 = wave_sum(hx.x + hx.y + hx.z + hx.w) * (1.0f / FIRA_D);
+    f32x4v o4 = (h - m1 - xh * m2) * rstd;
+    const size_t o = (size_t)row * FIRA_D + lane * 4;
+    *reinterpret_cast<f32x4v*>(f.ds + o) = o4;
+    if (f.p > 0.f) {
+        const uint32_t e0 = (uint32_t)row * FIRA_D + lane * 4;
+        o4.x *= dropout_scale(f.seed, f.site, e0 + 0, f.p, f.inv_keep);
+        o4.y *= dropout_scale(f.seed, f.site, e0 + 1, f.p, f.inv_keep);
+        o4.z *= dropout_scale(f.seed, f.site, e0 + 2, f.p, f.inv_keep);
+        o4.w *= dropout_scale(f.seed, f.site, e0 + 3, f.p, f.inv_keep);
+    }
+    *reinterpret_cast<f32x4v*>(f.dx + o) = o4;
+    cs[2] += o4;
+    cs[3] += o4 * rw;
+}
+
+template <int COLS>
+__device__ __forceinline__ void ln_fold_park(float* scr, const f32x4v (&cs)[4], float* acc, int wave, int lane, int t) {
+    constexpr int VPR = COLS / 256, ROUNDS = 1024 / COLS;
+    static_assert(VPR >= 1 && VPR * ROUNDS == 4, "ln_fold_park: COLS = 256, 512 or 1024");
+#pragma unroll
+    for (int rd = 0; rd < ROUNDS; ++rd) {
+        if (rd > 0) lds_barrier();
+#pragma unroll
+        for (int v = 0; v < VPR; ++v) *reinterpret_cast<f32x4v*>(&scr[wave * COLS + v * 256 + lane * 4]) = cs[rd * VPR + v];
+        lds_barrier();
+        if (t < COLS) {
+            float s = 0.f;
+#pragma unroll
+            for (int w = 0; w < 16; ++w) s += scr[w * COLS + t];
+            acc[rd * COLS + t] += s;
+        }
+    }
+}
+__device__ __forceinline__ void ln_fold_store(const LnBwdFold& f, const float* acc, int t) {
+    f.part[(size_t)blockIdx.x * 4 * FIRA_D + t] = acc[t];
+}
+
+}
```
